# mcomunita/syncfusion

Hardware: AMD Instinct MI355X
Metric: U-Net denoise steps/sec (batch x 2 s@22.05 kHz) (higher is better)
Workload: dtype bf16; 1 GPU; BASELINE configs[1]: batch=8/GPU, 50-step DDIM (v-sampler) denoising of 2 s @ 22.05 kHz clips (L0=45056 = 44*1024, cropped to 44100), bf16, embedding_scale=1.0 (1 U-Net eval/step), dummy cond; this run timed 1568 consecutive sampler steps (the cost of a step does not depend on the schedule length); batch_per_gpu=8, L0=45056, hip_graph=True, weights_broadcast_bytes=0, gathered_clips=8

## Files before the change

include/syncfusion_amd.h:

```cpp
#ifndef SYNCFUSION_AMD_H
#define SYNCFUSION_AMD_H

#include <stdint.h>

#ifdef __cplusplus
extern "C" {
#endif

#define SF_MAX_DEPTH 12

enum {
  SF_OK = 0,
  SF_ERR_INVALID = 1,
  SF_ERR_MISSING_WEIGHT = 2,
  SF_ERR_SHAPE = 3,
  SF_ERR_HIP = 4,
  SF_ERR_WORKSPACE = 5,
  SF_ERR_UNSUPPORTED = 6
};

enum { SF_UP_NEAREST_CONV3 = 0, SF_UP_TRANSPOSE = 1 };
enum { SF_F32 = 0, SF_BF16 = 1, SF_F16 = 2, SF_F32X = 3 };

typedef struct {
// ... 24 lines not shown
  int32_t modulation_features;
  int32_t resnet_groups;
  int32_t dtype;
  int32_t upsample_mode;
  int32_t time_fourier_features, time_no_first_act, attention_out_bias;
} sf_unet_config;

typedef struct sf_unet sf_unet;

int sf_unet_create(const sf_unet_config *cfg, const sf_tensor *weights, int n_weights, void *stream, sf_unet **out);
void sf_unet_destroy(sf_unet *h);

int sf_unet_param_count(const sf_unet_config *cfg);
int sf_unet_param_name(const sf_unet_config *cfg, int index, char *name_out, int name_cap, int64_t *numel_out);

int64_t sf_unet_workspace_bytes(const sf_unet *h, int B, int L0, int two_pass);
int64_t sf_vsample_workspace_bytes(const sf_unet *h, int B, int L0, int two_pass, int num_steps);

int sf_unet_forward(sf_unet *h, const float *x, const float *sigma, const float *const *ctx, const float *emb,
                    int B, int L0, float embedding_scale, float *out, void *ws, int64_t ws_bytes, void *stream);

int sf_vsample(sf_unet *h, float *x_inout, const float *const *ctx, const float *emb, int B, int L0,
               int num_steps, float embedding_scale, int use_graph, void *ws, int64_t ws_bytes, void *stream);

int sf_unet_debug_enable(sf_unet *h, float *buf, int64_t cap_floats);
int sf_unet_debug_count(const sf_unet *h);
int sf_unet_debug_info(const sf_unet *h, int i, char *name_out, int name_cap, int64_t *offset, int64_t *rows, int32_t *cols);

int sf_unet_launch_count(const sf_unet *h);
int sf_unet_graph_captures(const sf_unet *h);
int sf_unet_set_branches(sf_unet *h, int n);
int sf_unet_profile_enable(sf_unet *h, int on);
int sf_unet_profile_count(const sf_unet *h);
int sf_unet_profile_get(const sf_unet *h, int i, char *name_out, int name_cap, float *ms, double *flops, double *bytes);
int sf_unet_profile_depth(const sf_unet *h, int i);

typedef struct {
  int32_t n_layers;
  int32_t in_channels;
  int32_t channels;
  int32_t multipliers[SF_MAX_DEPTH + 1];
  int32_t factors[SF_MAX_DEPTH];
  int32_t num_blocks[SF_MAX_DEPTH];
  int32_t resnet_groups;
  int32_t patch_size;
} sf_encoder1d_config;

typedef struct sf_encoder1d sf_encoder1d;

int sf_encoder1d_create(const sf_encoder1d_config *cfg, const sf_tensor *weights, int n_weights, void *stream, sf_encoder1d **out);
void sf_encoder1d_destroy(sf_encoder1d *h);
int64_t sf_encoder1d_workspace_bytes(const sf_encoder1d *h, int B, int L0);
int sf_encoder1d_forward(sf_encoder1d *h, const float *y, int B, int L0, float *const *xs_out,
                         void *ws, int64_t ws_bytes, void *stream);

typedef struct sf_onsetnet sf_onsetnet;

int sf_onsetnet_create(const sf_tensor *weights, int n_weights, int dtype, void *stream, sf_onsetnet **out);
void sf_onsetnet_destroy(sf_onsetnet *h);
int64_t sf_onsetnet_workspace_bytes(const sf_onsetnet *h, int N, int T, int H, int W);
int sf_onsetnet_forward(sf_onsetnet *h, const float *frames, int N, int T, int H, int W, float *logits,
                        void *ws, int64_t ws_bytes, void *stream);
int sf_onsetnet_debug_enable(sf_onsetnet *h, float *buf, int64_t cap_floats);
int sf_onsetnet_debug_count(const sf_onsetnet *h);
int sf_onsetnet_debug_info(const sf_onsetnet *h, int i, char *name_out, int name_cap, int64_t *offset, int64_t *rows, int32_t *cols);
int sf_onsetnet_debug_detail(sf_onsetnet *h, int enable, const int32_t *clips, int n_clips);
#define SF_ONSET_PATH_GEMM 0
#define SF_ONSET_PATH_GEMM_SPLIT 1
#define SF_ONSET_PATH_SP 2
#define SF_ONSET_PATH_TW 3
#define SF_ONSET_PATH_STEM 4
int sf_onsetnet_debug_path(const sf_onsetnet *h, int i);

int sf_onsets_to_track(const float *logits, int N, int T, const int32_t *start_frame ,
                       float frame_rate, float sample_rate, float threshold, float *track, int L, void *stream);

int sf_cut_prefix_crop(const float *gen, const float *y, int B, int C, int L, int cut_length, float *out, int32_t *first_onset,
                       void *stream);

typedef struct sf_resampler sf_resampler;
int sf_resampler_create(int orig_freq, int new_freq, int lowpass_filter_width, float rolloff, sf_resampler **out);
void sf_resampler_destroy(sf_resampler *h);
int sf_resampler_out_length(const sf_resampler *h, int L);
int sf_resampler_forward(sf_resampler *h, const float *x, int R, int L, float *out, void *stream);

typedef struct sf_augment_clip {
  int32_t top, left;
  int32_t order[4];
  float factor[4];
  int32_t mask;
  int32_t reserved;
} sf_augment_clip;
int64_t sf_frames_augment_workspace_bytes(int N, int T, int out_h, int out_w);
int sf_frames_augment(const uint8_t *frames, int N, int T, int H, int W, int resize_h, int resize_w, int out_h, int out_w,
                      const sf_augment_clip *table_host, const sf_augment_clip *table_dev, const float *mean3, const float *std3, float *out,
                      void *ws, int64_t ws_bytes, void *stream);
int sf_frames_preprocess(const uint8_t *frames, int N, int T, int H, int W, int out_h, int out_w, const float *mean3, const float *std3,
                         float *out, void *stream);
int sf_times_to_track(const double *times, const int32_t *clip_of, int n_times, double sample_rate, int B, int L, float *track, void *stream);

int sf_op_conv1d_cl(int dtype, const void *x, const float *w, const float *bias, const float *gamma, const float *beta,
                    int groups, float eps, const void *residual, int B, int L, int C, int N, int taps, int stride,
                    int pad, int upsample, void *out, void *ws, int64_t ws_bytes, void *stream);
int64_t sf_op_conv1d_bwd_workspace_bytes(int B, int L, int C, int N, int taps, int groups);
int sf_op_conv1d_bwd_cl(const float *x, const float *w, const float *gamma, const float *beta, int groups, float eps, const float *dy,
                        int B, int L, int C, int N, int taps, int pad, float *dx, float *dw, float *db, float *dgb, void *ws,
                        int64_t ws_bytes, void *stream);
int64_t sf_op_gn_silu_train_stats_floats(int B, int L, int C, int groups);
int sf_op_gn_silu_train(const float *x, const float *gamma, const float *beta, int groups, float eps, int B, int L, int C, float *act, float *stats,
                        void *stream);
int sf_op_conv1d_bwd_cl_act(const float *x, const float *act, const float *stats , const float *w, const float *gamma, const float *beta,
                            int groups, float eps, const float *dy, int B, int L, int C, int N, int taps, int pad, float *dx, float *dw, float *db,
                            float *dgb, void *ws, int64_t ws_bytes, void *stream);
int sf_op_conv1d_bwd_cl_x(int dtype, const float *x, const float *act, const float *stats, const float *w, const float *gamma, const float *beta,
                          int groups, float eps, const float *dy, int B, int L, int C, int N, int taps, int pad, float *dx, float *dw, float *db,
                          float *dgb, void *ws, int64_t ws_bytes, void *stream);
int64_t sf_op_conv1d_dgrad_pack_bytes(int C, int N, int taps);
int sf_op_conv1d_train_fwd(int dtype, const float *x, const float *w, const float *bias, const float *gamma, const float *beta, int groups, float eps,
                           const float *residual, int B, int L, int C, int N, int taps, int pad, float *out, void *dgrad_pack, int64_t dgrad_pack_bytes,
                           void *ws, int64_t ws_bytes, void *stream);
int sf_op_conv1d_bwd_cl_p(int dtype, const float *x, const float *act, const float *stats, const float *w, const void *dgrad_pack, const float *gamma,
                          const float *beta, int groups, float eps, const float *dy, const float *dx_add, int B, int L, int C, int N, int taps, int pad,
                          float *dx, float *dw, float *db, float *dgb, void *ws, int64_t ws_bytes, void *stream);
int sf_op_conv1d_train_images(int dtype, const float *w, int B, int L, int C, int N, int taps, int pad, int groups);
int sf_op_conv1d_variant(int dtype, int B, int L, int C, int N, int taps, int stride, int pad, int upsample, int groups, char *label, int label_bytes);
int sf_op_conv1d_bwd_variant(int dtype, int B, int L, int C, int N, int taps, int pad, char *label, int label_bytes);
int sf_train_pack_many(const void *desc_dev, int n_items, int total_tiles, void *stream);
int sf_op_conv1d_train_fwd_pk(int dtype, const float *x, const float *w, const float *fw, const void *fwx, const float *bias, const float *gamma,
                              const float *beta, int groups, float eps, const float *residual, int B, int L, int C, int N, int taps, int pad, float *out,
                              void *ws, int64_t ws_bytes, void *stream);
int sf_op_ln_modulate_bwd_add(const float *x, const float *scale_shift, const float *dy, const float *dx_add, float eps, int B, int L, int C, float *dx,
                              float *dss, void *ws, int64_t ws_bytes, void *stream);
int64_t sf_op_length_sums_workspace_bytes(int B, int L, int C);
int sf_op_length_sums(const float *x, const float *y , int B, int L, int C, float *out , void *ws, int64_t ws_bytes,
                      void *stream);
int64_t sf_op_ln_modulate_bwd_workspace_bytes(int B, int L, int C);
int sf_op_ln_modulate_bwd(const float *x, const float *scale_shift, const float *dy, float eps, int B, int L, int C, float *dx, float *dss,
                          void *ws, int64_t ws_bytes, void *stream);
int sf_op_attention_bwd(const float *q, const float *kv, const float *out, const float *dout, int B, int L, int heads, int head_dim, float *dq,
                        float *dkv, void *ws, int64_t ws_bytes, void *stream);
int sf_op_attention_fwd_lse(const float *q, const float *kv, int B, int L, int heads, int head_dim, float *out, float *lse, void *stream);
int sf_op_attention_fwd_lse_x(int dtype, const float *q, const float *kv, int B, int L, int heads, int head_dim, float *out, float *lse, void *stream);
int sf_op_attention_bwd_lse(const float *q, const float *kv, const float *out, const float *dout, const float *lse, int B, int L, int heads, int head_dim,
                            float *dq, float *dkv, void *ws, int64_t ws_bytes, void *stream);
int sf_op_attention_bwd_lse_x(int dtype, const float *q, const float *kv, const float *out, const float *dout, const float *lse, int B, int L, int heads,
                              int head_dim, float *dq, float *dkv, void *ws, int64_t ws_bytes, void *stream);
int sf_bench_conv1d(int dtype, int B, int L, int C, int N, int taps, int upsample, int path, int tile, int sk, int iters,
                    float *ms_out);
int64_t sf_op_resnet_mod_cb_workspace_bytes(int B, int L, int C);
int sf_op_resnet_mod_cb(int dtype, const void *x, const float *w1, const float *b1, const float *w2, const float *b2, const float *gn1_g,
                        const float *gn1_b, const float *gn2_g, const float *gn2_b, int groups, float eps_gn, const float *scale_shift,
                        float eps_ln, int B, int L, int C, int kb , void *h_out, void *m_out,
                        void *ws, int64_t ws_bytes, void *stream);
int64_t sf_op_inject_prenorm_proj_workspace_bytes(int B, int L, int C, int C2, int N);
int sf_op_inject_prenorm_proj(int dtype, const void *m, const void *ctx, const float *w_inj, const float *b_inj, const float *gamma,
                              const float *beta, float eps, const float *w_q, int B, int L, int C, int C2, int N, void *z_out, void *q_out,
                              int *fused_out, void *ws, int64_t ws_bytes, void *stream);
int sf_bench_conv_cb(int dtype, int B, int L, int C, int groups, int kb, int cold, int iters, float *ms );
int sf_op_gn_silu(int dtype, const void *x, const float *gamma, const float *beta, int groups, float eps, int B, int L, int C, void *out,
                  void *ws, int64_t ws_bytes, void *stream);
int sf_op_ln_modulate(int dtype, const void *x, const float *scale_shift , float eps,
                      int B, int L, int C, void *out, void *stream);
int sf_op_attention(int dtype, const void *q, const void *kv, int B, int L, int heads, int head_dim, void *out, void *stream);


typedef struct {
  int32_t N, T, Hi, Wi;
  int32_t cin, cin_ld;
  int32_t cout, cout_ld;
  int32_t kt, kh, kw;
  int32_t sh, sw;
  int32_t pt, ph, pw;
} sf_vconv_desc;
int64_t sf_op_vconv_workspace_bytes(const sf_vconv_desc *desc );
int sf_op_vconv_fwd(const sf_vconv_desc *desc, const float *x, const float *w, float *y, void *ws, int64_t ws_bytes, void *stream);
int sf_op_vconv_bwd(const sf_vconv_desc *desc, const float *x, const float *w, const float *dy, float *dx, float *dw, void *ws, int64_t ws_bytes,
                    void *stream);
int64_t sf_op_bn_train_workspace_bytes(int64_t rows, int C);
int sf_op_bn_train_fwd(const float *x, const float *res, int64_t rows, int C, int ld, const float *gamma, const float *beta, float eps, float momentum,
                       float *running_mean, float *running_var, int64_t *num_batches_tracked, int relu, float *y, float *save_mean, float *save_invstd,
                       void *ws, int64_t ws_bytes, void *stream);
int sf_op_bn_train_bwd(const float *x, const float *y, const float *dy, int64_t rows, int C, int ld, const float *gamma, const float *save_mean,
                       const float *save_invstd, float *dx, float *dres, float *dgamma, float *dbeta, void *ws, int64_t ws_bytes, void *stream);
int64_t sf_op_bn_sync_workspace_bytes(int64_t rows, int C);
int sf_op_bn_sync_stats(const float *x, int64_t rows, int C, int ld, float *local_stats, void *ws, int64_t ws_bytes, void *stream);
int sf_op_bn_sync_fwd_apply(const float *x, const float *res, int64_t rows, int C, int ld, const float *gathered_stats, const int64_t *row_counts, int world,
                            const float *gamma, const float *beta, float eps, float momentum, float *running_mean, float *running_var,
                            int64_t *num_batches_tracked, int relu, float *y, float *save_mean, float *save_invstd, void *ws, int64_t ws_bytes,
                            void *stream);
int sf_op_bn_sync_bwd_sums(const float *x, const float *y, const float *dy, int64_t rows, int C, int ld, const float *save_mean, const float *save_invstd,
                           float *local_sums, float *dgamma, float *dbeta, void *ws, int64_t ws_bytes, void *stream);
int sf_op_bn_sync_bwd_apply(const float *x, const float *y, const float *dy, int64_t rows, int C, int ld, const float *gathered_sums,
                            const int64_t *row_counts, int world, const float *gamma, const float *save_mean, const float *save_invstd, float *dx,
                            float *dres, void *ws, int64_t ws_bytes, void *stream);
int sf_op_video_to_cl(const float *x, int N, int C, int T, int H, int W, int ld, float *out, void *stream);
int sf_op_video_pool(const float *x, int64_t NT, int HW, int C, int ld, float *out, void *stream);
int sf_op_video_pool_bwd(const float *dout, int64_t NT, int HW, int C, int ld, float *dx, void *stream);

int64_t sf_op_onset_loss_workspace_bytes(int64_t n);
int sf_op_onset_bce_fwd(const float *z, const float *t, int64_t n, float *loss, float *stats, void *ws, int64_t ws_bytes, void *stream);
int sf_op_onset_bce_bwd(const float *z, const float *t, const float *stats, const float *g, int64_t n, float *dz, void *stream);
int sf_op_onset_metrics(const float *z, const float *t, int N, int T, float threshold, double *out, void *ws, int64_t ws_bytes, void *stream);

#define SF_OPTIM_CHUNK 16384
int64_t sf_optim_workspace_bytes(int total_chunks);
int sf_optim_adamw_step(const void *desc_dev, int n_tensors, int total_chunks, const void *hyper_dev, int n_groups, int clip, float *result_dev,
                        void *ws, int64_t ws_bytes, void *stream);

typedef struct sf_audio_features sf_audio_features;
enum { SF_PAD_CONSTANT = 0, SF_PAD_REFLECT = 1 };
int sf_audio_features_create(int n_fft, int hop, int n_mels, int pad_mode, const int32_t *first_bin , const int32_t *bin_count ,
                             const float *weights , int64_t n_weights, sf_audio_features **out);
void sf_audio_features_destroy(sf_audio_features *h);
int64_t sf_audio_features_workspace_bytes(const sf_audio_features *h, int B, int L);
int sf_logmel_forward(sf_audio_features *h, const float *wav, int B, int L, float amin, float top_db, float *mel_power, float *db, void *ws,
                      int64_t ws_bytes, void *stream);
int sf_onset_detect(sf_audio_features *h, const float *wav, int B, int L, float amin, float top_db, int lag, int pre_max, int post_max,
                    int pre_avg, int post_avg, int wait, float delta, int conf_interval, int capacity, float *envelope, int32_t *count,
                    int32_t *positions, float *confidence, float *strength, void *ws, int64_t ws_bytes, void *stream);

#ifdef __cplusplus
}
#endif
#endif
```

syncfusion_amd/_lib.py:

```python
from __future__ import annotations

import ctypes as C
import os
from typing import Dict, Iterable, List, Optional, Sequence, Tuple

import torch

SF_MAX_DEPTH = 12
SF_F32, SF_BF16, SF_F16, SF_F32X = 0, 1, 2, 3
UPSAMPLE_MODES = {"nearest": 0, "transpose": 1}
DTYPES = {"fp32": SF_F32, "float32": SF_F32, "f32": SF_F32, "bf16": SF_BF16, "bfloat16": SF_BF16, "fp16": SF_F16, "float16": SF_F16, "f16": SF_F16, "half": SF_F16,
          "fp32x": SF_F32X}

_HERE = os.path.dirname(os.path.abspath(__file__))
LIB_PATH = os.environ.get("SF_LIB_PATH") or os.path.join(_HERE, "lib", "libsyncfusion_amd.so")


class SfTensor(C.Structure):
    _fields_ = [("name", C.c_char_p), ("data", C.c_void_p), ("numel", C.c_int64)]


class UnetConfig(C.Structure):
    _fields_ = [
        ("n_layers", C.c_int32), ("in_channels", C.c_int32),
        ("channels", C.c_int32 * SF_MAX_DEPTH), ("factors", C.c_int32 * SF_MAX_DEPTH),
        ("items", C.c_int32 * SF_MAX_DEPTH), ("attentions", C.c_int32 * SF_MAX_DEPTH),
        ("cross_attentions", C.c_int32 * SF_MAX_DEPTH), ("context_channels", C.c_int32 * SF_MAX_DEPTH),
        ("attention_heads", C.c_int32), ("attention_features", C.c_int32),
        ("embedding_features", C.c_int32), ("embedding_max_length", C.c_int32),
        ("modulation_features", C.c_int32), ("resnet_groups", C.c_int32), ("dtype", C.c_int32),
        ("upsample_mode", C.c_int32),
        ("time_fourier_features", C.c_int32), ("time_no_first_act", C.c_int32), ("attention_out_bias", C.c_int32),
    ]


class EncoderConfig(C.Structure):
    _fields_ = [
        ("n_layers", C.c_int32), ("in_channels", C.c_int32), ("channels", C.c_int32),
        ("multipliers", C.c_int32 * (SF_MAX_DEPTH + 1)), ("factors", C.c_int32 * SF_MAX_DEPTH),
        ("num_blocks", C.c_int32 * SF_MAX_DEPTH), ("resnet_groups", C.c_int32), ("patch_size", C.c_int32),
    ]


class VConvDesc(C.Structure):
    _fields_ = [(n, C.c_int32) for n in ("N", "T", "Hi", "Wi", "cin", "cin_ld", "cout", "cout_ld", "kt", "kh", "kw", "sh", "sw", "pt", "ph", "pw")]


_P, _I, _L, _F = C.c_void_p, C.c_int, C.c_int64, C.c_float
SYMBOLS = {
    "sf_version": (C.c_char_p, []),
    "sf_last_error": (C.c_char_p, []),
    "sf_device_ok": (_I, []),
    "sf_clock_probe_start": (_I, [C.c_double, _P]),
    "sf_clock_probe_read": (_I, [C.POINTER(C.c_double)]),
    "sf_unet_create": (_I, [C.POINTER(UnetConfig), C.POINTER(SfTensor), _I, _P, C.POINTER(_P)]),
    "sf_unet_destroy": (None, [_P]),
    "sf_unet_param_count": (_I, [C.POINTER(UnetConfig)]),
    "sf_unet_param_name": (_I, [C.POINTER(UnetConfig), _I, C.c_char_p, _I, C.POINTER(_L)]),
    "sf_unet_workspace_bytes": (_L, [_P, _I, _I, _I]),
    "sf_vsample_workspace_bytes": (_L, [_P, _I, _I, _I, _I]),
    "sf_unet_forward": (_I, [_P, _P, _P, C.POINTER(_P), _P, _I, _I, _F, _P, _P, _L, _P]),
    "sf_vsample": (_I, [_P, _P, C.POINTER(_P), _P, _I, _I, _I, _F, _I, _P, _L, _P]),
    "sf_unet_debug_enable": (_I, [_P, _P, _L]),
    "sf_unet_debug_count": (_I, [_P]),
    "sf_unet_debug_info": (_I, [_P, _I, C.c_char_p, _I, C.POINTER(_L), C.POINTER(_L), C.POINTER(C.c_int32)]),
    "sf_unet_launch_count": (_I, [_P]),
    "sf_unet_graph_captures": (_I, [_P]),
    "sf_unet_set_branches": (_I, [_P, _I]),
    "sf_unet_profile_enable": (_I, [_P, _I]),
    "sf_unet_profile_count": (_I, [_P]),
    "sf_unet_profile_get": (_I, [_P, _I, C.c_char_p, _I, C.POINTER(C.c_float), C.POINTER(C.c_double), C.POINTER(C.c_double)]),
    "sf_unet_profile_depth": (_I, [_P, _I]),
    "sf_encoder1d_create": (_I, [C.POINTER(EncoderConfig), C.POINTER(SfTensor), _I, _P, C.POINTER(_P)]),
    "sf_encoder1d_destroy": (None, [_P]),
    "sf_encoder1d_workspace_bytes": (_L, [_P, _I, _I]),
    "sf_encoder1d_forward": (_I, [_P, _P, _I, _I, C.POINTER(_P), _P, _L, _P]),
    "sf_onsetnet_create": (_I, [C.POINTER(SfTensor), _I, _I, _P, C.POINTER(_P)]),
    "sf_onsetnet_destroy": (None, [_P]),
    "sf_onsetnet_workspace_bytes": (_L, [_P, _I, _I, _I, _I]),
    "sf_onsetnet_forward": (_I, [_P, _P, _I, _I, _I, _I, _P, _P, _L, _P]),
    "sf_onsetnet_debug_enable": (_I, [_P, _P, _L]),
    "sf_onsetnet_debug_count": (_I, [_P]),
    "sf_onsetnet_debug_detail": (_I, [_P, _I, C.POINTER(C.c_int32), _I]),
    "sf_onsetnet_debug_path": (_I, [_P, _I]),
    "sf_onsetnet_debug_info": (_I, [_P, _I, C.c_char_p, _I, C.POINTER(_L), C.POINTER(_L), C.POINTER(C.c_int32)]),
    "sf_onsets_to_track": (_I, [_P, _I, _I, _P, _F, _F, _F, _P, _I, _P]),
    "sf_frames_preprocess": (_I, [_P, _I, _I, _I, _I, _I, _I, _P, _P, _P, _P]),
    "sf_frames_augment_workspace_bytes": (_L, [_I, _I, _I, _I]),
    "sf_frames_augment": (_I, [_P, _I, _I, _I, _I, _I, _I, _I, _I, _P, _P, _P, _P, _P, _P, _L, _P]),
    "sf_times_to_track": (_I, [_P, _P, _I, C.c_double, _I, _I, _P, _P]),
    "sf_cut_prefix_crop": (_I, [_P, _P, _I, _I, _I, _I, _P, _P, _P]),
    "sf_resampler_create": (_I, [_I, _I, _I, _F, C.POINTER(_P)]),
    "sf_resampler_destroy": (None, [_P]),
    "sf_resampler_out_length": (_I, [_P, _I]),
    "sf_resampler_forward": (_I, [_P, _P, _I, _I, _P, _P]),
    "sf_op_conv1d_cl": (_I, [_I, _P, _P, _P, _P, _P, _I, _F, _P, _I, _I, _I, _I, _I, _I, _I, _I, _P, _P, _L, _P]),
    "sf_op_conv1d_bwd_workspace_bytes": (_L, [_I, _I, _I, _I, _I, _I]),
    "sf_op_conv1d_bwd_cl": (_I, [_P, _P, _P, _P, _I, _F, _P, _I, _I, _I, _I, _I, _I, _P, _P, _P, _P, _P, _L, _P]),
    "sf_op_conv1d_bwd_cl_act": (_I, [_P, _P, _P, _P, _P, _P, _I, _F, _P, _I, _I, _I, _I, _I, _I, _P, _P, _P, _P, _P, _L, _P]),
    "sf_op_conv1d_bwd_cl_x": (_I, [_I, _P, _P, _P, _P, _P, _P, _I, _F, _P, _I, _I, _I, _I, _I, _I, _P, _P, _P, _P, _P, _L, _P]),
    "sf_op_conv1d_dgrad_pack_bytes": (_L, [_I, _I, _I]),
    "sf_op_conv1d_train_fwd": (_I, [_I, _P, _P, _P, _P, _P, _I, _F, _P, _I, _I, _I, _I, _I, _I, _P, _P, _L, _P, _L, _P]),
    "sf_op_conv1d_bwd_cl_p": (_I, [_I, _P, _P, _P, _P, _P, _P, _P, _I, _F, _P, _P, _I, _I, _I, _I, _I, _I, _P, _P, _P, _P, _P, _L, _P]),
    "sf_op_conv1d_train_images": (_I, [_I, _P, _I, _I, _I, _I, _I, _I, _I]),
    "sf_op_conv1d_variant": (_I, [_I, _I, _I, _I, _I, _I, _I, _I, _I, _I, C.c_char_p, _I]),
    "sf_op_conv1d_bwd_variant": (_I, [_I, _I, _I, _I, _I, _I, _I, C.c_char_p, _I]),
    "sf_train_pack_many": (_I, [_P, _I, _I, _P]),
    "sf_op_conv1d_train_fwd_pk": (_I, [_I, _P, _P, _P, _P, _P, _P, _P, _I, _F, _P, _I, _I, _I, _I, _I, _I, _P, _P, _L, _P]),
    "sf_op_ln_modulate_bwd_add": (_I, [_P, _P, _P, _P, _F, _I, _I, _I, _P, _P, _P, _L, _P]),
    "sf_op_gn_silu_train_stats_floats": (_L, [_I, _I, _I, _I]),
    "sf_op_gn_silu_train": (_I, [_P, _P, _P, _I, _F, _I, _I, _I, _P, _P, _P]),
    "sf_op_ln_modulate_bwd_workspace_bytes": (_L, [_I, _I, _I]),
    "sf_op_ln_modulate_bwd": (_I, [_P, _P, _P, _F, _I, _I, _I, _P, _P, _P, _L, _P]),
    "sf_op_attention_bwd": (_I, [_P, _P, _P, _P, _I, _I, _I, _I, _P, _P, _P, _L, _P]),
    "sf_op_attention_fwd_lse": (_I, [_P, _P, _I, _I, _I, _I, _P, _P, _P]),
    "sf_op_attention_fwd_lse_x": (_I, [_I, _P, _P, _I, _I, _I, _I, _P, _P, _P]),
    "sf_op_attention_bwd_lse": (_I, [_P, _P, _P, _P, _P, _I, _I, _I, _I, _P, _P, _P, _L, _P]),
    "sf_op_attention_bwd_lse_x": (_I, [_I, _P, _P, _P, _P, _P, _I, _I, _I, _I, _P, _P, _P, _L, _P]),
    "sf_op_length_sums_workspace_bytes": (_L, [_I, _I, _I]),
    "sf_op_length_sums": (_I, [_P, _P, _I, _I, _I, _P, _P, _L, _P]),
    "sf_bench_conv1d": (_I, [_I, _I, _I, _I, _I, _I, _I, _I, _I, _I, _I, C.POINTER(C.c_float)]),
    "sf_op_gn_silu": (_I, [_I, _P, _P, _P, _I, _F, _I, _I, _I, _P, _P, _L, _P]),
    "sf_op_inject_prenorm_proj_workspace_bytes": (_L, [_I, _I, _I, _I, _I]),
    "sf_op_inject_prenorm_proj": (_I, [_I, _P, _P, _P, _P, _P, _P, _F, _P, _I, _I, _I, _I, _I, _P, _P, _P, _P, _L, _P]),
    "sf_op_resnet_mod_cb_workspace_bytes": (_L, [_I, _I, _I]),
    "sf_op_resnet_mod_cb": (_I, [_I, _P, _P, _P, _P, _P, _P, _P, _P, _P, _I, _F, _P, _F, _I, _I, _I, _I, _P, _P, _P, _L, _P]),
    "sf_bench_conv_cb": (_I, [_I, _I, _I, _I, _I, _I, _I, _I, C.POINTER(C.c_float)]),
    "sf_op_ln_modulate": (_I, [_I, _P, _P, _F, _I, _I, _I, _P, _P]),
    "sf_op_attention": (_I, [_I, _P, _P, _I, _I, _I, _I, _P, _P]),
    "sf_op_vconv_workspace_bytes": (_L, [C.POINTER(VConvDesc)]),
    "sf_op_vconv_fwd": (_I, [C.POINTER(VConvDesc), _P, _P, _P, _P, _L, _P]),
    "sf_op_vconv_bwd": (_I, [C.POINTER(VConvDesc), _P, _P, _P, _P, _P, _P, _L, _P]),
    "sf_op_bn_train_workspace_bytes": (_L, [_L, _I]),
    "sf_op_bn_train_fwd": (_I, [_P, _P, _L, _I, _I, _P, _P, _F, _F, _P, _P, _P, _I, _P, _P, _P, _P, _L, _P]),
    "sf_op_bn_train_bwd": (_I, [_P, _P, _P, _L, _I, _I, _P, _P, _P, _P, _P, _P, _P, _P, _L, _P]),
    "sf_op_bn_sync_workspace_bytes": (_L, [_L, _I]),
    "sf_op_bn_sync_stats": (_I, [_P, _L, _I, _I, _P, _P, _L, _P]),
    "sf_op_bn_sync_fwd_apply": (_I, [_P, _P, _L, _I, _I, _P, _P, _I, _P, _P, _F, _F, _P, _P, _P, _I, _P, _P, _P, _P, _L, _P]),
    "sf_op_bn_sync_bwd_sums": (_I, [_P, _P, _P, _L, _I, _I, _P, _P, _P, _P, _P, _P, _L, _P]),
    "sf_op_bn_sync_bwd_apply": (_I, [_P, _P, _P, _L, _I, _I, _P, _P, _I, _P, _P, _P, _P, _P, _P, _L, _P]),
    "sf_op_video_to_cl": (_I, [_P, _I, _I, _I, _I, _I, _I, _P, _P]),
    "sf_op_video_pool": (_I, [_P, _L, _I, _I, _I, _P, _P]),
    "sf_op_video_pool_bwd": (_I, [_P, _L, _I, _I, _I, _P, _P]),
    "sf_op_onset_loss_workspace_bytes": (_L, [_L]),
    "sf_op_onset_bce_fwd": (_I, [_P, _P, _L, _P, _P, _P, _L, _P]),
    "sf_op_onset_bce_bwd": (_I, [_P, _P, _P, _P, _L, _P, _P]),
    "sf_op_onset_metrics": (_I, [_P, _P, _I, _I, _F, _P, _P, _L, _P]),
    "sf_optim_workspace_bytes": (_L, [_I]),
    "sf_optim_adamw_step": (_I, [_P, _I, _I, _P, _I, _I, _P, _P, _L, _P]),
    "sf_audio_features_create": (_I, [_I, _I, _I, _I, _P, _P, _P, _L, C.POINTER(_P)]),
    "sf_audio_features_destroy": (None, [_P]),
    "sf_audio_features_workspace_bytes": (_L, [_P, _I, _I]),
    "sf_logmel_forward": (_I, [_P, _P, _I, _I, _F, _F, _P, _P, _P, _L, _P]),
    "sf_onset_detect": (_I, [_P, _P, _I, _I, _F, _F, _I, _I, _I, _I, _I, _I, _F, _I, _I, _P, _P, _P, _P, _P, _P, _L, _P]),
}

_lib: Optional[C.CDLL] = None


class SyncFusionAmdError(RuntimeError):
    pass


def load() -> C.CDLL:
    global _lib
    if _lib is not None:
        return _lib
    if not os.path.exists(LIB_PATH):
        raise SyncFusionAmdError(
            f"{LIB_PATH} is missing: build it with `python -c 'import __graft_entry__ as g; g.build()'` "
            "(or `make -C syncfusion_amd/csrc`).  There is no CPU fallback.")
    lib = C.CDLL(LIB_PATH)
    for name, (res, args) in SYMBOLS.items():
        fn = getattr(lib, name)
        fn.restype = res
        fn.argtypes = args
    _lib = lib
    return lib


def check(rc: int, what: str) -> None:
    if rc != 0:
        msg = load().sf_last_error()
        raise SyncFusionAmdError(f"{what} failed (code {rc}): {msg.decode() if msg else '?'}")


def require_gpu_tensor(t: torch.Tensor, where: str) -> None:
    if not t.is_cuda:
        raise SyncFusionAmdError(f"{where}: expected a tensor on an MI355X (cuda/hip) device, got {t.device}; "
                                 "this build has no CPU execution path")


def stream_ptr(device: torch.device) -> int:
    return int(torch.cuda.current_stream(device).cuda_stream)


def f32c(t: torch.Tensor) -> torch.Tensor:
    return t.detach().to(torch.float32).contiguous()


class TensorTable:

    def __init__(self, named: Iterable[Tuple[str, torch.Tensor]], device: torch.device):
        self.keep: List[torch.Tensor] = []
        self.names: List[bytes] = []
        items = list(named)
        self.array = (SfTensor * max(1, len(items)))()
        self.n = len(items)
        for i, (name, t) in enumerate(items):
            tt = f32c(t).to(device)
            self.keep.append(tt)
            self.names.append(name.encode())
            self.array[i].name = self.names[-1]
            self.array[i].data = tt.data_ptr()
            self.array[i].numel = tt.numel()


def ptr_array(tensors: Sequence[torch.Tensor]):
    arr = (C.c_void_p * len(tensors))()
    for i, t in enumerate(tensors):
        arr[i] = t.data_ptr()
    return arr
```

syncfusion_amd/csrc/capi_misc.cpp:

```cpp
#include <algorithm>
#include <cstring>
#include <cstdlib>
#include <cmath>
#include <exception>

#include "engine_common.h"

using namespace sf;

#define SF_API_BEGIN try {
#define SF_API_END                  \
  }                                 \
  catch (const EngineError &e) {    \
    return e.code;                  \
  }                                 \
  catch (const std::exception &e) { \
    set_error("%s", e.what());      \
    return SF_ERR_INVALID;          \
  }

extern "C" {

const char *sf_version(void) { return "syncfusion_amd 0.1.0 (gfx950)"; }
const char *sf_last_error(void) { return get_error(); }
// ... 372 lines not shown
  if (!ms_out || iters < 1) fail(SF_ERR_INVALID, "bad argument");
  const bool x3 = dtype == SF_F32X;
  if (x3) dtype = F32;
  const size_t es = dsize(dtype);
  const int K = taps * C, Lout = L * upsample, M = B * Lout;
  void *x = nullptr, *w = nullptr, *out = nullptr, *res = nullptr;
  float *bias = nullptr;
  SF_HIP(hipMalloc(&x, (size_t)B * L * C * es));
  const size_t wbytes = (size_t)N * K * es;
  int ncopy = 1;
  if (const char *e = tune_env("SF_BENCH_COLD")) {
    if (atoi(e) > 0) ncopy = (int)std::min<size_t>(1024, ((size_t)768 << 20) / wbytes + 1);
  }
  SF_HIP(hipMalloc(&w, wbytes * ncopy));
  SF_HIP(hipMalloc(&out, (size_t)M * N * es));
  SF_HIP(hipMalloc(&res, (size_t)M * N * es));
  SF_HIP(hipMalloc(&bias, N * sizeof(float)));
  SF_HIP(hipMemset(x, 0x3c, (size_t)B * L * C * es));
  SF_HIP(hipMemset(w, 0xbc, wbytes * ncopy));
  SF_HIP(hipMemset(res, 0x3d, (size_t)M * N * es));
  SF_HIP(hipMemset(bias, 0, N * sizeof(float)));
  ConvGemmArgs a;
  a.src = x;
  a.src_ld = C;
  a.w = w;
  a.bias = bias;
  a.N = N;
  a.K = K;
  a.cin = C;
  a.taps = taps;
  a.pad = taps / 2;
  while ((1 << a.up_shift) < upsample) ++a.up_shift;
  a.Lsrc = L;
  a.Lout = Lout;
  a.M = M;
  a.out = out;
  a.out_ld = N;
  a.n_store = N;
  a.res = res;
  a.res_ld = N;
  g_conv_gemm_force.path = path;
  g_conv_gemm_force.tile = tile;
  g_conv_gemm_force.sk = sk;
  hipEvent_t e0, e1;
  SF_HIP(hipEventCreate(&e0));
  SF_HIP(hipEventCreate(&e1));
  hipError_t err = hipSuccess;
  unsigned *sink = nullptr;
  void *wfr = nullptr;
  if (dtype != F32 && (K % 64) == 0 && K <= 2048 && (N % 32) == 0 && (C % 16) == 0 && !tune_env("SF_BENCH_NO_WFR")) {
    SF_HIP(hipMalloc(&wfr, wbytes * ncopy));
    SF_HIP(hipMemcpy(wfr, w, wbytes * ncopy, hipMemcpyDeviceToDevice));
    a.wfr = wfr;
  }
  void *wx = nullptr;
  if (x3) {
    if (K % 32) fail(SF_ERR_UNSUPPORTED, "fp32x needs K %% 32 == 0");
    SF_HIP(hipMalloc(&wx, wbytes * ncopy));
    for (int c = 0; c < ncopy; ++c)
      SF_HIP(launch_pack_wx(reinterpret_cast<const float *>(static_cast<char *>(w) + (size_t)c * wbytes), N, K, static_cast<char *>(wx) + (size_t)c * wbytes, nullptr));
    a.wx = wx;
  }
  for (int i = 0; i < 3 && err == hipSuccess; ++i) err = launch_conv_gemm(dtype, a, nullptr);
  if (err == hipSuccess) {
    SF_HIP(hipDeviceSynchronize());
    SF_HIP(hipEventRecord(e0, nullptr));
    int pre = 0;
    if (const char *e = tune_env("SF_BENCH_PREFETCH")) pre = atoi(e);
    if (pre > 0 && pre % 1000 == 0) fail(SF_ERR_INVALID, "SF_BENCH_PREFETCH=%d: the workgroup count (value mod 1000) must be >= 1", pre);
    if (pre > 0) SF_HIP(hipMalloc(reinterpret_cast<void **>(&sink), 64));
    for (int i = 0; i < iters && err == hipSuccess; ++i) {
      a.w = static_cast<char *>(w) + (size_t)(i % ncopy) * wbytes;
      if (wfr) a.wfr = static_cast<char *>(wfr) + (size_t)(i % ncopy) * wbytes;
      if (wx) a.wx = static_cast<char *>(wx) + (size_t)(i % ncopy) * wbytes;
      if (pre > 0) err = launch_touch(a.w, wbytes, pre % 1000, sink, nullptr);
      if (pre < 1000 && err == hipSuccess) err = launch_conv_gemm(dtype, a, nullptr);
    }
    SF_HIP(hipEventRecord(e1, nullptr));
    SF_HIP(hipEventSynchronize(e1));
    SF_HIP(hipEventElapsedTime(ms_out, e0, e1));
    *ms_out /= (float)iters;
  }
  g_conv_gemm_force = ConvGemmForce();
  (void)hipEventDestroy(e0);
  (void)hipEventDestroy(e1);
  for (void *p : {x, w, out, res, (void *)bias}) (void)hipFree(p);
  if (sink) (void)hipFree(sink);
  if (wfr) (void)hipFree(wfr);
  if (wx) (void)hipFree(wx);
  if (err != hipSuccess) fail(SF_ERR_UNSUPPORTED, "variant not applicable: %s", hipGetErrorString(err));
  return SF_OK;
  SF_API_END
}

int64_t sf_op_resnet_mod_cb_workspace_bytes(int B, int L, int C) {
  Workspace dry(nullptr, 0);
  const int64_t M = (int64_t)B * L;
  dry.alloc(2 * (int64_t)C * C * 3 * 4);
  dry.alloc(M * C * 4);
  dry.alloc(M * C * 4);
  dry.alloc((int64_t)(C / 128) * M * C * 4);
  dry.alloc((int64_t)B * 32 * 64 * 2 * 4);
  return dry.used();
}

int sf_op_resnet_mod_cb(int dtype, const void *x, const float *w1, const float *b1, const float *w2, const float *b2, const float *gn1_g,
                        const float *gn1_b, const float *gn2_g, const float *gn2_b, int groups, float eps_gn, const float *scale_shift, float eps_ln,
                        int B, int L, int C, int kb, void *h_out, void *m_out, void *ws, int64_t ws_bytes, void *stream) {
  SF_API_BEGIN
  if (kb != 1 && kb != 2) fail(SF_ERR_INVALID, "kb must be 1 or 2");
  if (!x || !w1 || !b1 || !w2 || !b2 || !gn1_g || !gn1_b || !gn2_g || !gn2_b || !m_out || !ws) fail(SF_ERR_INVALID, "null argument");
  if (!conv_cb_shape_ok(dtype, B, L, C, C, groups) || groups > 64) fail(SF_ERR_UNSUPPORTED, "shape outside the channel-block convolution's coverage");
  hipStream_t s = static_cast<hipStream_t>(stream);
  Workspace wk(ws, ws_bytes);
  const int64_t M = (int64_t)B * L;
  const int S = C / 128 / kb;
  if (kb == 2 && ((C / 128) % 2 || C / groups < 32)) fail(SF_ERR_UNSUPPORTED, "two channel blocks per workgroup need C a multiple of 256 and >= 32 channels per group");
  if (kb == 2 && dtype == SF_F32X) fail(SF_ERR_UNSUPPORTED, "the split-operand form takes one channel block per workgroup");
  const int64_t es = (int64_t)dsize(dtype);
  const int adt = dtype == SF_F32X ? (int)F32 : dtype;
  char *wp = static_cast<char *>(wk.alloc(2 * (int64_t)C * C * 3 * es));
  void *wp1 = wp, *wp2 = wp + (int64_t)C * C * 3 * es;
  void *act = wk.alloc(M * C * es);
  void *h = h_out ? h_out : wk.alloc(M * C * es);
  float *slab = static_cast<float *>(wk.alloc((int64_t)S * M * C * 4));
  float *stats = static_cast<float *>(wk.alloc((int64_t)B * 32 * 64 * 2 * 4));
  SF_HIP(launch_pack_conv_cb(dtype, w1, C, C, wp1, s));
  SF_HIP(launch_pack_conv_cb(dtype, w2, C, C, wp2, s));
  SF_HIP(launch_gn_silu(adt, x, C, B, L, C, groups, gn1_g, gn1_b, eps_gn, act, C, s));
  ConvCbArgs a;
  a.src = act;
  a.src_ld = C;
  a.wp = wp1;
  a.slab = slab;
  a.B = B;
  a.L = L;
  a.C = a.N = C;
  a.kb = kb;
  SF_HIP(launch_conv_cb(dtype, a, s));
  const CbGnPlan gp = cb_gn_plan(L);
  SF_HIP(launch_cb_reduce_gn(adt, slab, S, B, L, C, b1, h, C, groups, stats, gp, s));
  a.src = h;
  a.wp = wp2;
  a.pro = 1;
  a.G = groups;
  a.nch = gp.nch;
  a.chunk_rows = gp.chunk_rows;
  a.stats = stats;
  a.gamma = gn2_g;
  a.beta = gn2_b;
  a.eps = eps_gn;
  SF_HIP(launch_conv_cb(dtype, a, s));
  SF_HIP(launch_cb_reduce_ln(adt, slab, S, B, L, C, b2, x, C, scale_shift, 2 * C, eps_ln, m_out, C, s));
  return SF_OK;
  SF_API_END
}

int64_t sf_op_inject_prenorm_proj_workspace_bytes(int B, int L, int C, int C2, int N) {
  if (B < 1 || L < 1 || C < 32 || C2 < 0 || N < 8) return -1;
  const int64_t M = (int64_t)B * L, K1 = C + (C2 + 31) / 32 * 32;
  return (int64_t)C * K1 * 2 + (int64_t)N * C * 2 + M * C * 2 + M * (C / 32) * 8 + (int64_t)(2 * N + C) * 4 + 4096;
}

int sf_op_inject_prenorm_proj(int dtype, const void *m, const void *ctx, const float *w_inj, const float *b_inj, const float *gamma,
                              const float *beta, float eps, const float *w_q, int B, int L, int C, int C2, int N, void *z_out, void *q_out,
                              int *fused_out, void *ws, int64_t ws_bytes, void *stream) {
  SF_API_BEGIN
  if (!m || !w_inj || !b_inj || !gamma || !beta || !w_q || !z_out || !q_out || !ws) fail(SF_ERR_INVALID, "null argument");
  if (dtype != BF16 && dtype != F16) fail(SF_ERR_UNSUPPORTED, "16-bit dtypes only");
  if (C % 32 || C2 % 32 || N % 32 || (C2 > 0 && !ctx)) fail(SF_ERR_UNSUPPORTED, "C, C2 and N must be multiples of 32");
  const int64_t need = sf_op_inject_prenorm_proj_workspace_bytes(B, L, C, C2, N);
  if (need < 0 || ws_bytes < need) fail(SF_ERR_WORKSPACE, "workspace too small: need %lld bytes", (long long)need);
  hipStream_t s = static_cast<hipStream_t>(stream);
  Workspace wk(ws, ws_bytes);
  const int64_t M = (int64_t)B * L;
  const int K1 = C + C2;
  void *w1 = wk.alloc((int64_t)C * K1 * 2), *w2 = wk.alloc((int64_t)N * C * 2), *tmp = wk.alloc(M * C * 2);
  float *rowpart = static_cast<float *>(wk.alloc(M * (C / 32) * 8));
  float *bias2 = static_cast<float *>(wk.alloc((int64_t)N * 4)), *colsum = static_cast<float *>(wk.alloc((int64_t)N * 4));
  SF_HIP(launch_pack_rows(dtype, w_inj, C, K1, K1, nullptr, w1, K1, s));
  SF_HIP(launch_pack_rows(dtype, w_q, N, C, C, gamma, w2, C, s));
  SF_HIP(launch_fold_bias(w_q, N, C, beta, nullptr, bias2, s));
  SF_HIP(launch_row_sums(dtype, w2, N, C, colsum, s));
  ConvGemmArgs a;
  a.src = m;
  a.src_ld = C;
  a.src2 = ctx;
  a.src2_ld = C2;
  a.w = w1;
  a.bias = b_inj;
  a.M = (int)M;
  a.N = a.n_store = C;
  a.K = K1;
  a.cin = C;
  a.cin2 = C2;
  a.taps = 1;
  a.Lout = a.Lsrc = L;
  a.out = z_out;
  a.out_ld = C;
  a.res = m;
  a.res_ld = C;
  ConvGemmArgs q;
  q.src = z_out;
  q.src_ld = C;
  q.w = w2;
  q.bias = bias2;
  q.M = (int)M;
  q.N = q.n_store = N;
  q.K = q.cin = C;
  q.taps = 1;
  q.Lout = q.Lsrc = L;
  q.out = q_out;
  q.out_ld = N;
  ConvGemmArgs ar = a, ql = q;
  ar.rowpart_out = rowpart;
  ar.rowpart_nt = C / 32;
  ql.ln_part = rowpart;
  ql.ln_nt = C / 32;
  ql.ln_eps = eps;
  ql.ln_colsum = colsum;
  ar.mt_ln = ql.mt_ln = 1;
  const bool fused = conv_gemm_emits_rowpart(dtype, ar) && conv_gemm_ln_ok(dtype, ql);
  if (fused_out) *fused_out = fused ? 1 : 0;
  if (fused) {
    SF_HIP(launch_conv_gemm(dtype, ar, s));
    SF_HIP(launch_conv_gemm_ln(dtype, ql, s));
  } else {
    if (!conv_gemm_supported(dtype, a) || !conv_gemm_supported(dtype, q)) fail(SF_ERR_UNSUPPORTED, "shape outside the GEMM kernels' coverage");
    SF_HIP(launch_conv_gemm(dtype, a, s));
    SF_HIP(launch_ln_modulate(dtype, z_out, C, nullptr, 0, eps, B, L, C, tmp, C, s));
    q.src = tmp;
    SF_HIP(launch_conv_gemm(dtype, q, s));
  }
  return SF_OK;
  SF_API_END
}

int sf_bench_conv_cb(int dtype, int B, int L, int C, int groups, int kb, int cold, int iters, float *ms) {
  SF_API_BEGIN
  if (!ms || iters < 1 || (kb != 1 && kb != 2)) fail(SF_ERR_INVALID, "bad argument");
  if (!conv_cb_shape_ok(dtype, B, L, C, C, groups)) fail(SF_ERR_UNSUPPORTED, "shape outside the channel-block convolution's coverage");
  const int64_t M = (int64_t)B * L;
  const int S = C / 128 / kb;
  const size_t wbytes = (size_t)C * C * 3 * 2;
  int ncopy = 1;
  if (cold) ncopy = (int)std::min<size_t>(256, (768u << 20) / wbytes + 1);
  void *w = nullptr, *x = nullptr, *h = nullptr;
  float *slab = nullptr, *stats = nullptr, *vec = nullptr;
  SF_HIP(hipMalloc(&w, wbytes * ncopy));
  SF_HIP(hipMalloc(&x, M * C * 2));
  SF_HIP(hipMalloc(&h, M * C * 2));
  SF_HIP(hipMalloc(reinterpret_cast<void **>(&slab), (size_t)S * M * C * 4));
  SF_HIP(hipMalloc(reinterpret_cast<void **>(&stats), (size_t)B * 32 * 64 * 2 * 4));
  SF_HIP(hipMalloc(reinterpret_cast<void **>(&vec), (size_t)(4 * C + (size_t)B * 2 * C) * 4));
  SF_HIP(hipMemset(w, 0x11, wbytes * ncopy));
  SF_HIP(hipMemset(x, 0x3c, M * C * 2));
  SF_HIP(hipMemset(vec, 0, (size_t)(4 * C + (size_t)B * 2 * C) * 4));
  const CbGnPlan gp = cb_gn_plan(L);
  ConvCbArgs a;
  a.src = x;
  a.src_ld = C;
  a.slab = slab;
  a.B = B;
  a.L = L;
  a.C = a.N = C;
  a.kb = kb;
  a.G = groups;
  a.nch = gp.nch;
  a.chunk_rows = gp.chunk_rows;
  a.stats = stats;
  a.gamma = vec;
  a.beta = vec + C;
  hipEvent_t e0, e1;
  SF_HIP(hipEventCreate(&e0));
  SF_HIP(hipEventCreate(&e1));
  hipError_t err = hipSuccess;
  for (int which = 0; which < 4 && err == hipSuccess; ++which) {
    auto one = [&](int i) -> hipError_t {
      a.wp = static_cast<char *>(w) + (size_t)(i % ncopy) * wbytes;
      switch (which) {
        case 0: a.pro = 0; return launch_conv_cb(dtype, a, nullptr);
        case 1: return launch_cb_reduce_gn(dtype, slab, S, B, L, C, vec + 2 * C, h, C, groups, stats, gp, nullptr);
        case 2: a.pro = 1; return launch_conv_cb(dtype, a, nullptr);
        default: return launch_cb_reduce_ln(dtype, slab, S, B, L, C, vec + 2 * C, x, C, vec + 4 * C, 2 * C, 1e-6f, h, C, nullptr);
      }
    };
    for (int i = 0; i < 3 && err == hipSuccess; ++i) err = one(i);
    if (err != hipSuccess) break;
    SF_HIP(hipDeviceSynchronize());
    SF_HIP(hipEventRecord(e0, nullptr));
    for (int i = 0; i < iters && err == hipSuccess; ++i) err = one(i);
    SF_HIP(hipEventRecord(e1, nullptr));
    SF_HIP(hipEventSynchronize(e1));
    SF_HIP(hipEventElapsedTime(&ms[which], e0, e1));
    ms[which] /= (float)iters;
  }
  (void)hipEventDestroy(e0);
  (void)hipEventDestroy(e1);
  for (void *p : {w, x, h, (void *)slab, (void *)stats, (void *)vec}) (void)hipFree(p);
  if (err != hipSuccess) fail(SF_ERR_HIP, "launch failed: %s", hipGetErrorString(err));
  return SF_OK;
  SF_API_END
}

int sf_op_ln_modulate(int dtype, const void *x, const float *scale_shift, float eps, int B, int L, int C, void *out, void *stream) {
  SF_API_BEGIN
// ... 19 lines not shown
```

syncfusion_amd/csrc/conv_cb.hip:

```cpp
#include <cstdlib>

#include "common.h"
#include "kernels.h"

namespace sf {
namespace {

constexpr int KC = 128;
constexpr int KC_LOG2 = 7;
constexpr int NSLOT = 4;
constexpr unsigned OOB = 0x80000000u;

template <typename T> __device__ __forceinline__ Vec16<T> buf_ld16(__amdgpu_buffer_rsrc_t r, unsigned byte_off) {
  Vec16<T> v;
  u32x4 raw = __builtin_amdgcn_raw_buffer_load_b128(r, byte_off, 0, 0);
  v.v = __builtin_bit_cast(decltype(v.v), raw);
  return v;
}

__device__ __forceinline__ float part_count(bool tiles, int clip, int kc, int mtile, int L, int chunk_rows, int log2cpg) {
  const int c0 = clip * L;
  const int rows = tiles ? min((mtile + 1) * 32, c0 + L) - max(mtile * 32, c0) : min(chunk_rows, L - kc * chunk_rows);
  return (float)(rows << (tiles ? 5 : log2cpg));
}

__device__ __forceinline__ float2 merge_parts(const float2 (&cs)[4], const float (&cn)[4], int sub, int lim, float rn, float eps) {
  float s1 = 0.f;
#pragma unroll
  for (int k = 0; k < 4; ++k)
    if (sub + 8 * k < lim) s1 = fmaf(cn[k], cs[k].x, s1);
  const float mean = sum8_dpp(s1) * rn;
  float s2 = 0.f;
#pragma unroll
  for (int k = 0; k < 4; ++k)
    if (sub + 8 * k < lim) {
      const float d = cs[k].x - mean;
      s2 += fmaf(cn[k] * d, d, cs[k].y);
    }
  return make_float2(mean, rsqrtf(sum8_dpp(s2) * rn + eps));
}

template <typename T, int MT, bool PRO, int KB>
__global__ __launch_bounds__(256) void conv_cb_kernel(const ConvCbArgs a, const int mtiles, const unsigned bytes_src) {
  using frag = typename Frag16<T>::type;
  constexpr int KCW = KC * KB, PITCHW = KCW + 8, TPR = KCW / 8, RPP = 256 / TPR;
  constexpr int BM = 32 * MT, PR = BM + 2, NV = (PR + RPP - 1) / RPP;
  __shared__ __attribute__((aligned(16))) T panel[PR * PITCHW];
  __shared__ float2 gstat[NSLOT][8];
  const int tid = threadIdx.x, lane = tid & 63;
  const int wave = __builtin_amdgcn_readfirstlane(tid >> 6);
  const int nws = (int)gridDim.x;
  if ((int)blockIdx.y >= mtiles) {
    prefetch_slice(a.pf, ((int)blockIdx.y - mtiles) * nws + (int)blockIdx.x, 256);
    return;
  }
  const int mt = (int)blockIdx.y, ws = (int)blockIdx.x;
  const int nt = ws >> a.log2S, cb = ws & ((1 << a.log2S) - 1);
  const int r0 = mt * BM, M = a.B * a.L;
  auto divL = [&](int x) { return (int)__umulhi((unsigned)x, a.magicL); };

  const __amdgpu_buffer_rsrc_t rS = __builtin_amdgcn_make_buffer_rsrc(const_cast<void *>(a.src), 0, bytes_src, 0x00020000);
  const int cv = tid % TPR, pr = tid / TPR;
  Vec16<T> pv[NV];
  const unsigned col_b = (unsigned)((cb * KCW + cv * 8) * sizeof(T)), row_b = (unsigned)(a.src_ld * sizeof(T));
#pragma unroll
  for (int i = 0; i < NV; ++i) {
    const int j = pr + RPP * i, r = r0 - 1 + j;
    const bool ok = j < PR && r >= 0 && r < M;
    pv[i] = buf_ld16<T>(rS, ok ? (unsigned)r * row_b + col_b : OOB);
  }
  const int gshift = KC_LOG2 + (KB == 2 ? 1 : 0) - a.log2cpg;
  const int clip0 = divL(max(r0 - 1, 0));
  const int nclip = PRO ? (divL(min(r0 + BM, M - 1)) - clip0 + 1) : 0;
  const int npair = nclip << gshift;
  f32x4 ga[2], be[2];
  constexpr int NRD = 1;
  float2 cs[NRD][4];
  float cn[NRD][4];
  int lim[NRD] = {0};
  const int sub = tid & 7;
  if constexpr (PRO) {
    const int G = a.C >> a.log2cpg;
#pragma unroll
    for (int q = 0; q < 2; ++q) {
      ga[q] = *reinterpret_cast<const f32x4 *>(a.gamma + cb * KCW + cv * 8 + 4 * q);
      be[q] = *reinterpret_cast<const f32x4 *>(a.beta + cb * KCW + cv * 8 + 4 * q);
    }
    const bool tiles = a.pro == 2;
    const int ltpg = a.log2cpg - 5, ct = a.C >> 5;
#pragma unroll
    for (int rd = 0; rd < NRD; ++rd) {
      const int p = min((tid >> 3) + 32 * rd, npair - 1);
      const int slot = p >> gshift, gi = p & ((1 << gshift) - 1);
      const int clip = clip0 + slot;
      const int mt_lo = (clip * a.L) >> 5, nmt = ((clip * a.L + a.L - 1) >> 5) - mt_lo + 1;
      lim[rd] = tiles ? (nmt << max(ltpg, 0)) : a.nch;
#pragma unroll
      for (int k = 0; k < 4; ++k) {
        const int kc = min(sub + 8 * k, lim[rd] - 1);
        const int mtile = mt_lo + (kc >> max(ltpg, 0));
        const int tile = (((cb << gshift) + gi) << max(ltpg, 0)) + (kc & ((1 << max(ltpg, 0)) - 1));
        const unsigned off2 = (unsigned)(((mtile * ct + tile) * 2 + (clip - divL(mtile << 5))) * 2);
        const unsigned off1 = (unsigned)((((clip * a.nch + kc) * G) + (cb << gshift) + gi) * 2);
        cs[rd][k] = *reinterpret_cast<const float2 *>(a.stats + (tiles ? off2 : off1));
        cn[rd][k] = part_count(tiles, clip, kc, mtile, a.L, a.chunk_rows, a.log2cpg);
      }
    }
  }
  __builtin_amdgcn_sched_barrier(0);
  frag wf[24 * KB];
#pragma unroll
  for (int blk = 0; blk < KB; ++blk) {
    const frag *wp = reinterpret_cast<const frag *>(a.wp) + ((size_t)((cb * KB + blk) * (a.N >> 5) + (nt * 4 + wave)) * 24) * 64;
#pragma unroll
    for (int s = 0; s < 24; ++s) wf[blk * 24 + s] = wp[s * 64 + lane];
  }
  __builtin_amdgcn_sched_barrier(0);
  if constexpr (PRO) {
#pragma unroll
    for (int rd = 0; rd < NRD; ++rd)
#pragma unroll
      for (int k = 0; k < 4; ++k) asm volatile("" : "+v"(cs[rd][k].x), "+v"(cs[rd][k].y));
  }
  if constexpr (PRO) {
    const float rn = 1.0f / ((float)a.L * (float)(1 << a.log2cpg));
#pragma unroll
    for (int rd = 0; rd < NRD; ++rd) {
      const float2 st = merge_parts(cs[rd], cn[rd], sub, lim[rd], rn, a.eps);
      const int p = (tid >> 3) + 32 * rd;
      if (sub == 0 && p < npair) gstat[p >> gshift][p & ((1 << gshift) - 1)] = st;
    }
    __syncthreads();
  }
#pragma unroll
  for (int i = 0; i < NV; ++i) {
    const int j = pr + RPP * i, r = r0 - 1 + j;
    if (j < PR) {
      Vec16<T> o = pv[i];
      if (PRO && r >= 0 && r < M) {
        const float2 st = gstat[divL(r) - clip0][(cv * 8) >> a.log2cpg];
#pragma unroll
        for (int e = 0; e < 8; ++e) {
          const float sc = st.y * ga[e >> 2][e & 3];
          const float sh = fmaf(-st.x, sc, be[e >> 2][e & 3]);
          o.set(e, silu_t<true>(fmaf(pv[i].get(e), sc, sh)));
        }
      }
      st16<T>(panel + j * PITCHW + cv * 8, o);
    }
  }
  __syncthreads();
  const int fr = lane & 31, fh = lane >> 5;
  bool ok0[MT], ok2[MT];
#pragma unroll
  for (int t = 0; t < MT; ++t) {
    const int m = r0 + t * 32 + fr, l = m - divL(m) * a.L;
    ok0[t] = l > 0;
    ok2[t] = l < a.L - 1;
  }
  f32x16 acc[MT];
#pragma unroll
  for (int t = 0; t < MT; ++t)
#pragma unroll
    for (int r = 0; r < 16; ++r) acc[t][r] = 0.f;
  const frag zf = __builtin_bit_cast(frag, u32x4{0u, 0u, 0u, 0u});
#pragma unroll
  for (int blk = 0; blk < KB; ++blk)
#pragma unroll
    for (int tap = 0; tap < 3; ++tap)
#pragma unroll
      for (int ks = 0; ks < 8; ++ks)
#pragma unroll
        for (int t = 0; t < MT; ++t) {
          frag af = *reinterpret_cast<const frag *>(panel + (t * 32 + fr + tap) * PITCHW + blk * KC + ks * 16 + fh * 8);
          if (tap == 0) af = ok0[t] ? af : zf;
          if (tap == 2) af = ok2[t] ? af : zf;
          acc[t] = mfma32x16(wf[blk * 24 + tap * 8 + ks], af, acc[t]);
        }
  float *sl = a.slab + (size_t)cb * M * a.N + nt * 128 + wave * 32 + 4 * fh;
#pragma unroll
  for (int t = 0; t < MT; ++t) {
    const int m = r0 + t * 32 + fr;
    if (m < M) {
#pragma unroll
      for (int g = 0; g < 4; ++g) {
        f32x4 v = {acc[t][4 * g], acc[t][4 * g + 1], acc[t][4 * g + 2], acc[t][4 * g + 3]};
        *reinterpret_cast<f32x4 *>(sl + (unsigned)(m * a.N + 8 * g)) = v;
      }
    }
  }
}

template <int MT, bool PRO>
__global__ __launch_bounds__(256) void conv_cb_x3_kernel(const ConvCbArgs a, const int mtiles, const unsigned bytes_src) {
  using frag = f16x8;
  constexpr int PITCHW = KC + 8, TPR = KC / 4, RPP = 256 / TPR;
  constexpr int BM = 32 * MT, PR = BM + 2, NV = (PR + RPP - 1) / RPP;
  __shared__ __attribute__((aligned(16))) f16 panelH[PR * PITCHW], panelL[PR * PITCHW];
  __shared__ float2 gstat[NSLOT][8];
  const int tid = threadIdx.x, lane = tid & 63;
  const int wave = __builtin_amdgcn_readfirstlane(tid >> 6);
  const int nws = (int)gridDim.x;
  if ((int)blockIdx.y >= mtiles) {
    prefetch_slice(a.pf, ((int)blockIdx.y - mtiles) * nws + (int)blockIdx.x, 256);
    return;
  }
  const int mt = (int)blockIdx.y, ws = (int)blockIdx.x;
  const int nt = ws >> a.log2S, cb = ws & ((1 << a.log2S) - 1);
  const int r0 = mt * BM, M = a.B * a.L;
  auto divL = [&](int x) { return (int)__umulhi((unsigned)x, a.magicL); };

  const __amdgpu_buffer_rsrc_t rS = __builtin_amdgcn_make_buffer_rsrc(const_cast<void *>(a.src), 0, bytes_src, 0x00020000);
  const int cv = tid % TPR, pr = tid / TPR;
  f32x4 pv[NV];
  const unsigned col_b = (unsigned)((cb * KC + cv * 4) * 4), row_b = (unsigned)(a.src_ld * 4);
#pragma unroll
  for (int i = 0; i < NV; ++i) {
    const int j = pr + RPP * i, r = r0 - 1 + j;
    const bool ok = j < PR && r >= 0 && r < M;
    pv[i] = __builtin_bit_cast(f32x4, __builtin_amdgcn_raw_buffer_load_b128(rS, ok ? (unsigned)r * row_b + col_b : OOB, 0, 0));
  }
  const int gshift = KC_LOG2 - a.log2cpg;
  const int clip0 = divL(max(r0 - 1, 0));
  const int nclip = PRO ? (divL(min(r0 + BM, M - 1)) - clip0 + 1) : 0;
  const int npair = nclip << gshift;
  f32x4 ga = {1.f, 1.f, 1.f, 1.f}, be = {0.f, 0.f, 0.f, 0.f};
  float2 cs[4];
  float cn[4];
  int lim = 0;
  const int sub = tid & 7;
  if constexpr (PRO) {
    const int G = a.C >> a.log2cpg;
    ga = *reinterpret_cast<const f32x4 *>(a.gamma + cb * KC + cv * 4);
    be = *reinterpret_cast<const f32x4 *>(a.beta + cb * KC + cv * 4);
    const bool tiles = a.pro == 2;
    const int ltpg = a.log2cpg - 5, ct = a.C >> 5;
    const int p = min(tid >> 3, npair - 1);
    const int slot = p >> gshift, gi = p & ((1 << gshift) - 1);
    const int clip = clip0 + slot;
    const int mt_lo = (clip * a.L) >> 5, nmt = ((clip * a.L + a.L - 1) >> 5) - mt_lo + 1;
    lim = tiles ? (nmt << max(ltpg, 0)) : a.nch;
#pragma unroll
    for (int k = 0; k < 4; ++k) {
      const int kc = min(sub + 8 * k, lim - 1);
      const int mtile = mt_lo + (kc >> max(ltpg, 0));
      const int tile = (((cb << gshift) + gi) << max(ltpg, 0)) + (kc & ((1 << max(ltpg, 0)) - 1));
      const unsigned off2 = (unsigned)(((mtile * ct + tile) * 2 + (clip - divL(mtile << 5))) * 2);
      const unsigned off1 = (unsigned)((((clip * a.nch + kc) * G) + (cb << gshift) + gi) * 2);
      cs[k] = *reinterpret_cast<const float2 *>(a.stats + (tiles ? off2 : off1));
      cn[k] = part_count(tiles, clip, kc, mtile, a.L, a.chunk_rows, a.log2cpg);
    }
  }
  __builtin_amdgcn_sched_barrier(0);
  frag wh[24], wl[24];
  {
    const frag *wp = reinterpret_cast<const frag *>(a.wp) + ((size_t)(cb * (a.N >> 5) + (nt * 4 + wave)) * 48) * 64;
#pragma unroll
    for (int s = 0; s < 24; ++s) {
      wh[s] = wp[(2 * s) * 64 + lane];
      wl[s] = wp[(2 * s + 1) * 64 + lane];
    }
  }
  __builtin_amdgcn_sched_barrier(0);
  if constexpr (PRO) {
#pragma unroll
    for (int k = 0; k < 4; ++k) asm volatile("" : "+v"(cs[k].x), "+v"(cs[k].y));
  }
  if constexpr (PRO) {
    const float rn = 1.0f / ((float)a.L * (float)(1 << a.log2cpg));
    const float2 st = merge_parts(cs, cn, sub, lim, rn, a.eps);
    const int p = tid >> 3;
    if (sub == 0 && p < npair) gstat[p >> gshift][p & ((1 << gshift) - 1)] = st;
    __syncthreads();
  }
  typedef f16 f16x4_c __attribute__((ext_vector_type(4)));
#pragma unroll
  for (int i = 0; i < NV; ++i) {
    const int j = pr + RPP * i, r = r0 - 1 + j;
    if (j < PR) {
      f32x4 o = pv[i];
      if (PRO && r >= 0 && r < M) {
        const float2 st = gstat[divL(r) - clip0][(cv * 4) >> a.log2cpg];
#pragma unroll
        for (int e = 0; e < 4; ++e) {
          const float sc = st.y * ga[e];
          const float sh = fmaf(-st.x, sc, be[e]);
          o[e] = silu_t<false>(fmaf(pv[i][e], sc, sh));
        }
      }
      f16x4_c h, l;
#pragma unroll
      for (int e = 0; e < 4; ++e) {
        f16 x, y;
        x3_split1<X3_F16>(o[e], x, y);
        h[e] = x;
        l[e] = y;
      }
      *reinterpret_cast<f16x4_c *>(panelH + j * PITCHW + cv * 4) = h;
      *reinterpret_cast<f16x4_c *>(panelL + j * PITCHW + cv * 4) = l;
    }
  }
  __syncthreads();
  const int fr = lane & 31, fh = lane >> 5;
  bool ok0[MT], ok2[MT];
#pragma unroll
  for (int t = 0; t < MT; ++t) {
    const int m = r0 + t * 32 + fr, l = m - divL(m) * a.L;
    ok0[t] = l > 0;
    ok2[t] = l < a.L - 1;
  }
  f32x16 acc[MT], accL[MT];
#pragma unroll
  for (int t = 0; t < MT; ++t)
#pragma unroll
    for (int r = 0; r < 16; ++r) acc[t][r] = accL[t][r] = 0.f;
  const frag zf = __builtin_bit_cast(frag, u32x4{0u, 0u, 0u, 0u});
#pragma unroll
  for (int tap = 0; tap < 3; ++tap)
#pragma unroll
    for (int ks = 0; ks < 8; ++ks)
#pragma unroll
      for (int t = 0; t < MT; ++t) {
        const int o = (t * 32 + fr + tap) * PITCHW + ks * 16 + fh * 8;
        frag ah = *reinterpret_cast<const frag *>(panelH + o), al = *reinterpret_cast<const frag *>(panelL + o);
        if (tap == 0) {
          ah = ok0[t] ? ah : zf;
          al = ok0[t] ? al : zf;
        }
        if (tap == 2) {
          ah = ok2[t] ? ah : zf;
          al = ok2[t] ? al : zf;
        }
        x3_mfma<X3_F16>(wh[tap * 8 + ks], wl[tap * 8 + ks], ah, al, acc[t], accL[t]);
      }
  float *sl = a.slab + (size_t)cb * M * a.N + nt * 128 + wave * 32 + 4 * fh;
#pragma unroll
  for (int t = 0; t < MT; ++t) {
    const int m = r0 + t * 32 + fr;
    if (m < M) {
#pragma unroll
      for (int g = 0; g < 4; ++g) {
        f32x4 v;
// ... 65 lines not shown
  const f32x4 bi = *reinterpret_cast<const f32x4 *>(bias + c);
  float xs[P][4];
  float s1 = 0.f;
#pragma unroll
  for (int p = 0; p < P; ++p) {
    const int lr = p * 8 + rr;
    f32x4 x = v[p][0];
#pragma unroll
    for (int s = 1; s < S; ++s) x += v[p][s];
    x += bi;
    T o[4];
#pragma unroll
    for (int e = 0; e < 4; ++e) {
      o[e] = from_f<T>(x[e]);
      xs[p][e] = lr < rows ? to_f(o[e]) : 0.f;
      s1 += xs[p][e];
    }
    if (lr < rows) __builtin_memcpy(__builtin_assume_aligned(out + ((size_t)b * L + l0 + lr) * out_ld + c, 4 * sizeof(T)), o, 4 * sizeof(T));
  }
  const int cpg = N / G, span = cpg / 4;
  const int gpb = 128 / cpg;
  auto group_total = [&](float t, int k) {
    for (int off = 1; off < span; off <<= 1) t += __shfl_xor(t, off, 64);
    t += __shfl_xor(t, 32, 64);
    if (lane < 32 && (cq % span) == 0) red[wave][cq / span][k] = t;
    __syncthreads();
    float a = 0.f;
    if (tid < gpb) {
#pragma unroll
      for (int w = 0; w < 4; ++w) a += red[w][tid][k];
    }
    return a;
  };
  const float a1 = group_total(s1, 0);
  if (tid < gpb) gmean[tid] = a1 / ((float)rows * (float)cpg);
  __syncthreads();
  const float mu = gmean[cq / span];
  float s2 = 0.f;
#pragma unroll
  for (int p = 0; p < P; ++p) {
    const bool live = p * 8 + rr < rows;
#pragma unroll
    for (int e = 0; e < 4; ++e) {
      const float d = live ? xs[p][e] - mu : 0.f;
      s2 = fmaf(d, d, s2);
    }
  }
  const float a2 = group_total(s2, 1);
  if (tid < gpb) {
    float *o = stats + (((size_t)b * nch + ch) * G + cblk * gpb + tid) * 2;
    o[0] = gmean[tid];
    o[1] = a2;
  }
}

template <typename T, int S, int TPR>
__global__ __launch_bounds__(256) void cb_reduce_ln_kernel(const float *__restrict__ slab, const int M, const int C, const int L,
                                                           const float *__restrict__ bias, const T *__restrict__ res, const int res_ld,
                                                           const float *__restrict__ ss, const int ss_ld, const float eps, T *__restrict__ out,
                                                           const int out_ld, const int nreal, const Prefetch pf) {
  constexpr int RPB = 256 / TPR, WPR = TPR >= 64 ? TPR / 64 : 1;
  __shared__ float red[2][4];
  if ((int)blockIdx.x >= nreal) {
    prefetch_slice(pf, (int)blockIdx.x - nreal, 256);
    return;
  }
  const int tid = threadIdx.x, wave = tid >> 6;
  const int row = (int)blockIdx.x * RPB + tid / TPR, sub = tid % TPR;
  const bool active = row < M;
  const size_t m = active ? row : 0;
  const int c = sub * 4, b = (int)(m / L);
  f32x4 v[S];
#pragma unroll
  for (int s = 0; s < S; ++s) v[s] = *reinterpret_cast<const f32x4 *>(slab + ((size_t)s * M + m) * C + c);
  T rv[4];
  __builtin_memcpy(rv, __builtin_assume_aligned(res + m * res_ld + c, 4 * sizeof(T)), 4 * sizeof(T));
  const f32x4 bi = *reinterpret_cast<const f32x4 *>(bias + c);
  f32x4 sc = {0.f, 0.f, 0.f, 0.f}, sh = {0.f, 0.f, 0.f, 0.f};
  if (ss) {
    sc = *reinterpret_cast<const f32x4 *>(ss + (size_t)b * ss_ld + c);
    sh = *reinterpret_cast<const f32x4 *>(ss + (size_t)b * ss_ld + C + c);
  }
  f32x4 y = v[0];
#pragma unroll
  for (int s = 1; s < S; ++s) y += v[s];
  y += bi;
#pragma unroll
  for (int e = 0; e < 4; ++e) y[e] += to_f(rv[e]);
  auto row_sum = [&](float x, int slot) {
    constexpr int W = TPR < 64 ? TPR : 64;
#pragma unroll
    for (int o = W >> 1; o > 0; o >>= 1) x += __shfl_xor(x, o, 64);
    if constexpr (WPR > 1) {
      if ((tid & 63) == 0) red[slot][wave] = x;
      __syncthreads();
      const int w0 = (wave / WPR) * WPR;
      x = 0.f;
#pragma unroll
      for (int w = 0; w < WPR; ++w) x += red[slot][w0 + w];
    }
    return x;
  };
  const float mean = row_sum((y[0] + y[1]) + (y[2] + y[3]), 0) / (float)C;
  float q = 0.f;
#pragma unroll
  for (int e = 0; e < 4; ++e) {
    const float d = y[e] - mean;
    q = fmaf(d, d, q);
  }
  const float rstd = rsqrtf(row_sum(q, 1) / (float)C + eps);
  if (!active) return;
  T o[4];
#pragma unroll
  for (int e = 0; e < 4; ++e) {
    float z = (y[e] - mean) * rstd;
    if (ss) z = fmaf(z, 1.0f + sc[e], sh[e]);
    o[e] = from_f<T>(z);
  }
  __builtin_memcpy(__builtin_assume_aligned(out + (size_t)row * out_ld + c, 4 * sizeof(T)), o, 4 * sizeof(T));
}

int cb_min_wgs() {
  static const int v = [] {
    const char *e = tune_env("SF_CB_MIN_WGS");
    return e && atoi(e) > 0 ? atoi(e) : 160;
  }();
  return v;
}

}

size_t conv_cb_weight_elems(int N, int C) { return (size_t)N * C * 3; }

bool conv_cb_shape_ok(int dt, int B, int L, int C, int N, int G) {
  if (dt == F32) return false;
  if (C < KC || (C % KC) || (N % 128) || C / KC > 8 || ((C / KC) & (C / KC - 1))) return false;
  if (L < 44 || (int64_t)B * L * (int64_t)(C > N ? C : N) * 4 >= 0x7FFFFFF0ll) return false;
  if ((uint64_t)B * L * (uint64_t)L >= (1ull << 32)) return false;
  if (G > 0) {
    if (C % G) return false;
    const int cpg = C / G;
    if (cpg < 16 || cpg > KC || (cpg & (cpg - 1))) return false;
  }
  return true;
}

bool conv_cb_tile_stats_ok(int L, int C, int G) {
  if (G < 1 || C % G) return false;
  const int cpg = C / G;
  if (cpg < 32 || (cpg & (cpg - 1)) || L < 32) return false;
  return ((L + 30) / 32 + 1) * (cpg / 32) <= 32;
}

int conv_cb_mt(int M, int N, int C) {
  static const int forced = [] {
    const char *e = tune_env("SF_CB_MT");
    return e ? atoi(e) : 0;
  }();
  if (forced >= 1 && forced <= 4) return forced;
  const int nws = (N / 128) * (C / KC);
  return ((M + 63) / 64) * nws >= cb_min_wgs() ? 2 : 1;
}

hipError_t launch_pack_conv_cb(int dt, const float *w, int N, int C, void *out, hipStream_t s) {
  if (dt == F32 || (C % KC) || (N % 32)) return hipErrorInvalidValue;
  const size_t total = (size_t)N * C * 3;
  const int blocks = (int)std::min<size_t>((total + 255) / 256, 4096);
  if (dt == F32X) hipLaunchKernelGGL(pack_conv_cb_x3_kernel, dim3(blocks), dim3(256), 0, s, w, N, C, static_cast<f16 *>(out));
  else if (dt == BF16) hipLaunchKernelGGL((pack_conv_cb_kernel<bf16>), dim3(blocks), dim3(256), 0, s, w, N, C, static_cast<bf16 *>(out));
  else hipLaunchKernelGGL((pack_conv_cb_kernel<f16>), dim3(blocks), dim3(256), 0, s, w, N, C, static_cast<f16 *>(out));
  return hipGetLastError();
}

hipError_t launch_conv_cb(int dt, const ConvCbArgs &a0, hipStream_t s) {
  if (!conv_cb_shape_ok(dt, a0.B, a0.L, a0.C, a0.N, a0.pro ? a0.G : 0)) return hipErrorInvalidValue;
  if (a0.pro == 1 && a0.nch > 32) return hipErrorInvalidValue;
  if (a0.pro == 2 && !conv_cb_tile_stats_ok(a0.L, a0.C, a0.G)) return hipErrorInvalidValue;
  ConvCbArgs a = a0;
  if (dt == F32X && a.kb == 2) return hipErrorInvalidValue;
  const int kb = a.kb == 2 ? 2 : 1;
  const int M = a.B * a.L, S = a.C / KC / kb;
  if (kb == 2 && ((a.C / KC) % 2 || (a.pro && a.C / a.G < 32))) return hipErrorInvalidValue;
  a.log2S = 0;
  while ((1 << a.log2S) < S) ++a.log2S;
  const int cpg = a.pro ? a.C / a.G : KC;
  a.log2cpg = 0;
  while ((1 << a.log2cpg) < cpg) ++a.log2cpg;
  if ((1 << a.log2S) != S || (1 << a.log2cpg) != cpg) return hipErrorInvalidValue;
  a.magicL = (unsigned)((0x100000000ull + (unsigned)a.L - 1) / (unsigned)a.L);
  int mt = kb == 2 ? std::min(2, conv_cb_mt(M, a.N, a.C / 2)) : conv_cb_mt(M, a.N, a.C);
  if (dt == F32X) mt = std::min(mt, 2);
  const int mtiles = (M + 32 * mt - 1) / (32 * mt), nws = (a.N / 128) * S;
  const int pf_rows = (a.pf.ptr && a.pf.bytes >= 16 && a.pf.wgs > 0) ? (a.pf.wgs + nws - 1) / nws : 0;
  a.pf.wgs = pf_rows * nws;
  const dim3 grid(nws, mtiles + pf_rows);
  const unsigned bytes_src = (unsigned)((size_t)M * a.src_ld * dsize(dt));
  if (dt == F32X) {
    if (a.pro) {
      if (mt == 1) hipLaunchKernelGGL((conv_cb_x3_kernel<1, true>), grid, dim3(256), 0, s, a, mtiles, bytes_src);
      else hipLaunchKernelGGL((conv_cb_x3_kernel<2, true>), grid, dim3(256), 0, s, a, mtiles, bytes_src);
    } else {
      if (mt == 1) hipLaunchKernelGGL((conv_cb_x3_kernel<1, false>), grid, dim3(256), 0, s, a, mtiles, bytes_src);
      else hipLaunchKernelGGL((conv_cb_x3_kernel<2, false>), grid, dim3(256), 0, s, a, mtiles, bytes_src);
    }
    return hipGetLastError();
  }
#define SF_CB2(T, MT, KB_)                                                                                                \
  do {                                                                                                                    \
    if (a.pro) hipLaunchKernelGGL((conv_cb_kernel<T, MT, true, KB_>), grid, dim3(256), 0, s, a, mtiles, bytes_src);       \
    else hipLaunchKernelGGL((conv_cb_kernel<T, MT, false, KB_>), grid, dim3(256), 0, s, a, mtiles, bytes_src);            \
  } while (0)
#define SF_CB(T, MT)                 \
  do {                               \
    if (kb == 2) SF_CB2(T, MT, 2);   \
    else SF_CB2(T, MT, 1);           \
  } while (0)
#define SF_CB_T(T)            \
  switch (mt) {               \
    case 1: SF_CB(T, 1); break; \
    case 2: SF_CB(T, 2); break; \
    case 3: if (kb == 2) { SF_CB2(T, 2, 2); } else { SF_CB2(T, 3, 1); } break; \
    default: if (kb == 2) { SF_CB2(T, 2, 2); } else { SF_CB2(T, 4, 1); } break; \
  }
  if (dt == BF16) { SF_CB_T(bf16) } else { SF_CB_T(f16) }
#undef SF_CB_T
#undef SF_CB
#undef SF_CB2
  return hipGetLastError();
}

CbGnPlan cb_gn_plan(int L) {
  CbGnPlan p;
  int P = 1;
  while (P < 4 && (L + 8 * P - 1) / (8 * P) > 32) P *= 2;
  p.chunk_rows = 8 * P;
  p.nch = (L + p.chunk_rows - 1) / p.chunk_rows;
  return p;
}

hipError_t launch_cb_reduce_gn(int dt, const float *slab, int S, int B, int L, int N, const float *bias, void *out, int out_ld, int G, float *stats,
                               const CbGnPlan &gp, hipStream_t s, Prefetch pf) {
  if ((N % 128) || N % G || (N / G) < 16 || (N / G) > 128 || (128 % (N / G)) || gp.nch > 32 || (out_ld % 4)) return hipErrorInvalidValue;
  const int P = gp.chunk_rows / 8, M = B * L;
  const int nreal = B * gp.nch * (N / 128);
  const dim3 grid(nreal + (pf.ptr && pf.bytes >= 16 ? pf.wgs : 0));
#define SF_RG(T, S_, P_)                                                                                                                          \
  hipLaunchKernelGGL((cb_reduce_gn_kernel<T, S_, P_>), grid, dim3(256), 0, s, slab, M, N, L, bias, static_cast<T *>(out), out_ld, G, stats, gp.nch, \
                     nreal, pf)
#define SF_RG_P(T, S_)            \
  switch (P) {                    \
    case 1: SF_RG(T, S_, 1); break; \
    case 2: SF_RG(T, S_, 2); break; \
    case 4: SF_RG(T, S_, 4); break; \
    default: return hipErrorInvalidValue; \
  }
#define SF_RG_S(T)                \
  switch (S) {                    \
    case 1: SF_RG_P(T, 1) break;  \
    case 2: SF_RG_P(T, 2) break;  \
    case 4: SF_RG_P(T, 4) break;  \
    case 8: SF_RG_P(T, 8) break;  \
    default: return hipErrorInvalidValue; \
  }
  if (dt == BF16) { SF_RG_S(bf16) } else if (dt == F16) { SF_RG_S(f16) } else { SF_RG_S(float) }
#undef SF_RG_S
#undef SF_RG_P
#undef SF_RG
  return hipGetLastError();
}

hipError_t launch_cb_reduce_ln(int dt, const float *slab, int S, int B, int L, int C, const float *bias, const void *res, int res_ld, const float *ss,
                               int ss_ld, float eps, void *out, int out_ld, hipStream_t s, Prefetch pf) {
  const int tpr = C / 4;
  if ((C % 128) || (tpr != 32 && tpr != 64 && tpr != 128 && tpr != 256) || (res_ld % 4) || (out_ld % 4)) return hipErrorInvalidValue;
  if (ss && ((ss_ld % 4) || (reinterpret_cast<uintptr_t>(ss) % 16))) return hipErrorInvalidValue;
  const int M = B * L, rpb = 256 / tpr;
  const int nreal = (M + rpb - 1) / rpb;
  const dim3 grid(nreal + (pf.ptr && pf.bytes >= 16 ? pf.wgs : 0));
#define SF_RL(T, S_, TPR_)                                                                                                                     \
  hipLaunchKernelGGL((cb_reduce_ln_kernel<T, S_, TPR_>), grid, dim3(256), 0, s, slab, M, C, L, bias, static_cast<const T *>(res), res_ld, ss, ss_ld, \
                     eps, static_cast<T *>(out), out_ld, nreal, pf)
#define SF_RL_T(T, S_)               \
  switch (tpr) {                     \
    case 32: SF_RL(T, S_, 32); break;  \
    case 64: SF_RL(T, S_, 64); break;  \
    case 128: SF_RL(T, S_, 128); break; \
    default: SF_RL(T, S_, 256); break; \
  }
#define SF_RL_S(T)                 \
  switch (S) {                     \
    case 1: SF_RL_T(T, 1) break;   \
    case 2: SF_RL_T(T, 2) break;   \
    case 4: SF_RL_T(T, 4) break;   \
    case 8: SF_RL_T(T, 8) break;   \
    default: return hipErrorInvalidValue; \
  }
  if (dt == BF16) { SF_RL_S(bf16) } else if (dt == F16) { SF_RL_S(f16) } else { SF_RL_S(float) }
#undef SF_RL_S
#undef SF_RL_T
#undef SF_RL
  return hipGetLastError();
}

}
```

syncfusion_amd/csrc/conv_gemm.hip:

```cpp
#include <cstring>
#include <set>
#include <string>

#include "common.h"
#include "kernels.h"

namespace sf {

namespace {

constexpr int BK = 32;

template <typename T> struct Lds {
  static constexpr int LD = BK + 16 / (int)sizeof(T);
};

struct RowState {
  int valid_m;
  int b_rel;
  int p0;
  int base;
  int t, h, w;
};

// ... 274 lines not shown
        rv[r] = has_res ? to_f(res[(size_t)m * a.res_ld + nc]) : 0.f;
        const int b = has_b ? m / a.Lout : 0;
        sv[r] = has_bs ? a.bscale[(size_t)b * a.bscale_ld + nc] : 1.f;
        av[r] = has_ba ? a.badd[(size_t)b * a.badd_ld + nc] : 0.f;
      }
#pragma unroll
      for (int r = 0; r < 16; ++r) {
        const int m = m0 + wr * WTM + i * 32 + (r & 3) + 8 * (r >> 2) + 4 * fh;
        float v = (acc[i][j][r] + bias) * sv[r] + rv[r] + av[r];
        v = real ? apply_act(v, a.act) : 0.f;
        if (m < a.M && n < a.n_store) {
          if (a.out_f32) static_cast<float *>(a.out)[(size_t)m * a.out_ld + n] = v;
          else out[(size_t)m * a.out_ld + n] = from_f<T>(v);
        }
      }
    }
  }
}

template <typename T, int BM, int BN, int WM_, int WN_, bool SC>
hipError_t launch_cfg(const ConvGemmArgs &a, hipStream_t s) {
  constexpr int LD = Lds<T>::LD;
  size_t lds = (size_t)(BM + BN) * LD * sizeof(T);
  if (a.pro == 1) {
    int nb = min(a.M / a.Lout + (a.M % a.Lout ? 1 : 0), BM / a.Lout + 2);
    lds += (size_t)nb * (a.cin + a.G) * sizeof(float2);
  }
  dim3 grid((a.M + BM - 1) / BM, (a.n_store + BN - 1) / BN);
  auto kern = conv_gemm_kernel<T, BM, BN, WM_, WN_, SC>;
  static bool big_lds_enabled = false;
  if (!big_lds_enabled) {
    hipError_t e = hipFuncSetAttribute(reinterpret_cast<const void *>(kern), hipFuncAttributeMaxDynamicSharedMemorySize, 128 * 1024);
    if (e != hipSuccess) return e;
    big_lds_enabled = true;
  }
  hipLaunchKernelGGL(kern, grid, dim3(256), lds, s, a);
  return hipGetLastError();
}

int pick_variant(const ConvGemmArgs &a);
int pick_variant(const ConvGemmArgs &a) {
  if (g_conv_gemm_force.path == 1 && g_conv_gemm_force.tile >= 1 && g_conv_gemm_force.tile <= 4) return g_conv_gemm_force.tile;
  const bool scalar_a = (a.cin % BK) != 0 || (a.cin2 % BK) != 0;
  if (scalar_a) return (a.cin2 != 0 || a.pro != 0) ? -1 : 0;
  const long M = a.M, N = a.n_store;
  auto blocks = [&](int bm, int bn) { return ((M + bm - 1) / bm) * ((N + bn - 1) / bn); };
  if (N <= 32) return 1;
  if (N <= 64) return blocks(128, 64) >= 512 ? 2 : 3;
  if (blocks(128, 128) >= 512) return 4;
  if (blocks(128, 64) >= 384) return 2;
  return 3;
}

template <typename T> hipError_t dispatch(const ConvGemmArgs &a, hipStream_t s) {
  switch (pick_variant(a)) {
    case 0: return launch_cfg<T, 64, 64, 2, 2, true>(a, s);
    case 1: return launch_cfg<T, 128, 32, 4, 1, false>(a, s);
    case 2: return launch_cfg<T, 128, 64, 2, 2, false>(a, s);
    case 3: return launch_cfg<T, 64, 64, 2, 2, false>(a, s);
    case 4: return launch_cfg<T, 128, 128, 2, 2, false>(a, s);
    default: return hipErrorInvalidValue;
  }
}

}

bool conv_gemm_supported(int dt, const ConvGemmArgs &a) {
  (void)dt;
  if (a.M <= 0 || a.N <= 0 || a.K <= 0) return false;
  if (a.pro == 1) {
    if (a.geom != 0 || a.cin % BK || a.cin % a.G) return false;
    int nb = min(a.M / a.Lout + 1, 128 / a.Lout + 2);
    if ((size_t)nb * (a.cin + a.G) * 8 > 96 * 1024) return false;
  }
  return true;
}

hipError_t launch_conv_gemm_sk(int dt, const ConvGemmArgs &a, hipStream_t s);
int conv_gemm_sk_variant(const ConvGemmArgs &a);
bool conv_gemm_fast_ok(int dt, const ConvGemmArgs &a);
bool conv_gemm_wp_ok(int dt, const ConvGemmArgs &a);
bool conv_gemm_prefers_wp(const ConvGemmArgs &a);

static bool use_sk(const ConvGemmArgs &a) {
  const int v = pick_variant(a);
  if (v <= 0 || (a.K % 32)) return false;
  static const int bm[5] = {64, 128, 128, 64, 128}, bn[5] = {64, 32, 64, 64, 128};
  const long blocks = (long)((a.M + bm[v] - 1) / bm[v]) * ((a.n_store + bn[v] - 1) / bn[v]);
  return blocks < 256 && a.K >= 256;
}

const char *label_for_dtype(int dt, const char *bf16_label) {
  if (dt != F16) return bf16_label;
  static std::set<std::string> pool;
  std::string s(bf16_label);
  const size_t at = s.find("bf16");
  if (at != std::string::npos) s.replace(at, 4, "f16");
  return pool.insert(s).first->c_str();
}

static const char *variant_name_bf16(int dt, const ConvGemmArgs &a);
static const char *label_x3(const ConvGemmArgs &a, const char *f32_label) {
  if (!a.wx) return f32_label;
  std::string s(f32_label);
  if (s.rfind("conv_gemm_wp<f32", 0) != 0 && s.rfind("conv_gemm_fast<f32", 0) != 0) return f32_label;
  static std::set<std::string> pool;
  s.replace(s.find("f32"), 3, "x3");
  return pool.insert(s).first->c_str();
}
const char *conv_gemm_variant_name(int dt, const ConvGemmArgs &a) {
  return dt == F32 ? label_x3(a, variant_name_bf16(dt, a)) : label_for_dtype(dt, variant_name_bf16(dt, a));
}
bool conv_gemm_reads_split_only(int dt, const ConvGemmArgs &a_in) {
  ConvGemmArgs a = a_in;
  a.w = a.wx = reinterpret_cast<const void *>(16);
  return std::strstr(conv_gemm_variant_name(dt, a), "<x3") != nullptr;
}

static long short_act_tiles() {
  static const long v = [] {
    const char *e = tune_env("SF_SHORT_TILES");
    const long t = e ? atol(e) : 0;
    return t > 0 ? t : 500L;
  }();
  return v;
}

bool conv_gemm_prefers_mt(const ConvGemmArgs &a) {
  static const int mode = [] {
    const char *e = tune_env("SF_MT");
    return e ? atoi(e) : 1;
  }();
  if (mode == 0) return false;
  if (mode == 2) return true;
  static const int min_tiles = [] {
    const char *e = tune_env("SF_MT_TILES");
    const int v = e ? atoi(e) : 0;
    return v > 0 ? v : 40;
  }();
  if (a.n_store <= 64 && a.geom != 1) return false;
  const long tiles = (long)((a.M + 127) / 128) * ((a.n_store + 127) / 128);
  return tiles >= 2 * min_tiles && a.K >= (a.geom == 1 ? 128 : 256);
}

static const char *variant_name_bf16(int dt, const ConvGemmArgs &a) {
  if (g_conv_gemm_force.path == 6 || (g_conv_gemm_force.path == 0 && conv_gemm_mt_wanted(dt, a))) return dt == F32 ? (a.wx ? "conv_gemm_mt<x3>" : "conv_gemm_mt<f32>") : conv_gemm_mt_name(a);
  static const char *names[2][5] = {{"conv_gemm<f32,64x64,scalarA>", "conv_gemm<f32,128x32>", "conv_gemm<f32,128x64>", "conv_gemm<f32,64x64>", "conv_gemm<f32,128x128>"},
                                    {"conv_gemm<bf16,64x64,scalarA>", "conv_gemm<bf16,128x32>", "conv_gemm<bf16,128x64>", "conv_gemm<bf16,64x64>", "conv_gemm<bf16,128x128>"}};
  static const char *sk_names[2][3] = {{"conv_gemm_sk<f32,64x64>", "conv_gemm_sk<f32,64x32>", "conv_gemm_sk<f32,32x32>"},
                                       {"conv_gemm_sk<bf16,64x64>", "conv_gemm_sk<bf16,64x32>", "conv_gemm_sk<bf16,32x32>"}};
  static const char *fast_names[2][3] = {{"conv_gemm_fast<f32,64x64>", "conv_gemm_fast<f32,64x32>", "conv_gemm_fast<f32,32x32>"},
                                         {"conv_gemm_fast<bf16,64x64>", "conv_gemm_fast<bf16,64x32>", "conv_gemm_fast<bf16,32x32>"}};
  const long t64 = (long)((a.M + 63) / 64) * ((a.n_store + 63) / 64);
  const bool short_act = t64 < short_act_tiles() && a.K >= 256 && (a.K % 32) == 0 && (a.cin % 32) == 0 && (a.cin2 % 32) == 0;
  if (!short_act) {
    V2Plan pl;
    if (conv_gemm_v2_plan(dt, a, pl)) return conv_gemm_v2_name(dt, pl);
  }
  static const char *wp_names[2][3] = {{"conv_gemm_wp<f32,32x32>", "conv_gemm_wp<f32,32x32>", "conv_gemm_wp<f32,32x32>"},
                                       {"conv_gemm_wp<bf16,64x64>", "conv_gemm_wp<bf16,64x32>", "conv_gemm_wp<bf16,32x32>"}};
  if ((short_act || use_sk(a)) && conv_gemm_prefers_wp(a) && conv_gemm_sk_variant(a) == 2 && g_conv_gemm_force.path == 0 && conv_gemm_rs_ok(dt, a))
    return dt == F32 ? "conv_gemm_rs<x3,32x32>" : "conv_gemm_rs<bf16,32x32>";
  if ((short_act || use_sk(a)) && conv_gemm_prefers_wp(a) && conv_gemm_wp_ok(dt, a)) return wp_names[dt == F32 ? 0 : 1][conv_gemm_sk_variant(a)];
  if (short_act || use_sk(a)) return (conv_gemm_fast_ok(dt, a) ? fast_names : sk_names)[dt == F32 ? 0 : 1][conv_gemm_sk_variant(a)];
  int v = pick_variant(a);
  return v < 0 ? "conv_gemm<invalid>" : names[dt == F32 ? 0 : 1][v];
}

ConvGemmForce g_conv_gemm_force;


bool conv_gemm_emits_rowpart(int dt, const ConvGemmArgs &a) {
  if (g_conv_gemm_force.path != 0 || !conv_gemm_supported(dt, a)) return false;
  {
    ConvGemmArgs plain = a;
    plain.rowpart_out = nullptr;
    if (conv_gemm_mt_wanted(dt, plain)) {
      const bool off = a.mt_ln == 0;
      ConvGemmArgs probe = a;
      if (!probe.rowpart_out) {
        probe.rowpart_out = reinterpret_cast<float *>(16);
        probe.rowpart_nt = a.n_store / 32;
      }
      return !off && conv_gemm_mt_wanted(dt, probe);
    }
  }
  if ((a.n_store % 32) || a.n_store != a.N) return false;
  const long t64 = (long)((a.M + 63) / 64) * ((a.n_store + 63) / 64);
  const bool short_act = t64 < short_act_tiles() && a.K >= 256 && (a.K % 32) == 0 && (a.cin % 32) == 0 && (a.cin2 % 32) == 0;
  if (!(short_act || use_sk(a))) return false;
  if ((a.cin % 32) || (a.cin2 % 32) || (a.K % 32)) return false;
  if (conv_gemm_sk_variant(a) != 2) return false;
  const bool prefer_wp = conv_gemm_prefers_wp(a);
  if (prefer_wp && conv_gemm_wp_ok(dt, a)) return true;
  return conv_gemm_fast_ok(dt, a);
}

bool conv_gemm_emits_gnpart(int dt, const ConvGemmArgs &a) {
  ConvGemmArgs plain = a;
  plain.gnpart_out = nullptr;
  if (a.geom != 0 || a.Lout < 32 || !conv_gemm_emits_rowpart(dt, plain)) return false;
  return conv_gemm_prefers_wp(a) && conv_gemm_wp_ok(dt, a);
}

hipError_t launch_conv_gemm(int dt, const ConvGemmArgs &a, hipStream_t s) {
  if (!conv_gemm_supported(dt, a)) return hipErrorInvalidValue;
  if (a.src_x3 && (dt != F32 || g_conv_gemm_force.path != 0 || !conv_gemm_src_x3_ok(a))) return hipErrorInvalidValue;
  const ConvGemmForce &f = g_conv_gemm_force;
  if (f.path == 6) return launch_conv_gemm_mt(dt, a, s);
  if (f.path == 0 && conv_gemm_mt_wanted(dt, a)) return launch_conv_gemm_mt(dt, a, s);
  const long t64 = (long)((a.M + 63) / 64) * ((a.n_store + 63) / 64);
  const bool short_act = t64 < short_act_tiles() && a.K >= 256 && (a.K % 32) == 0 && (a.cin % 32) == 0 && (a.cin2 % 32) == 0;
  if (f.path == 4 || (f.path == 0 && !short_act)) {
    V2Plan pl;
    if (conv_gemm_v2_plan(dt, a, pl)) return launch_conv_gemm_v2(dt, a, pl, s);
    if (f.path == 4) return hipErrorInvalidValue;
  }
  if (f.path == 2 || f.path == 5 || (f.path == 0 && (short_act || use_sk(a)))) return launch_conv_gemm_sk(dt, a, s);
  return SF_DISPATCH_T(dt, dispatch<T>(a, s));
}

}
```

syncfusion_amd/csrc/kernels.h:

```cpp
#pragma once
#include <hip/hip_runtime.h>
#include <stdint.h>

#include <cstdlib>

namespace sf {

#ifdef SF_TUNING_HOOKS
inline const char *tune_env(const char *name) { return getenv(name); }
#else
inline const char *tune_env(const char *) { return nullptr; }
#endif

enum DType { F32 = 0, BF16 = 1, F16 = 2, F32X = 3 };
constexpr int X3_F16 = 1, X3_BF16 = 2;
inline size_t dsize(int dt) { return (dt == F32 || dt == F32X) ? 4 : 2; }
#define SF_DISPATCH_T(dt, EXPR_T)             \
  ((dt) == ::sf::F32    ? [&] { using T = float; return EXPR_T; }()   \
   : (dt) == ::sf::BF16 ? [&] { using T = ::sf::bf16; return EXPR_T; }() \
                        : [&] { using T = ::sf::f16; return EXPR_T; }())
#define SF_DISPATCH_STMT(dt, STMT)                                   \
  do {                                                               \
    if ((dt) == ::sf::F32) { using T = float; STMT; }                \
    else if ((dt) == ::sf::BF16) { using T = ::sf::bf16; STMT; }     \
    else { using T = ::sf::f16; STMT; }                              \
  } while (0)

struct Prefetch {
  const void *ptr = nullptr;
  unsigned bytes = 0;
  int wgs = 0;
};

struct ConvGemmArgs {
  Prefetch pf;
  const void *src = nullptr, *src2 = nullptr, *w = nullptr, *res = nullptr;
  const void *wfr = nullptr;
  const float *w32 = nullptr;
  const void *wx = nullptr;
  const void *wfrx = nullptr;
  int wx_mode = 1;
  int src_x3 = 0;
  int solo = 0;
  void *out = nullptr;
  const float *bias = nullptr, *gamma = nullptr, *beta = nullptr, *stats = nullptr;
  const float *badd = nullptr, *bscale = nullptr;
  int M = 0, N = 0, K = 0;
  int cin = 0, cin2 = 0, src_ld = 0, src2_ld = 0, out_ld = 0, res_ld = 0, n_store = 0;
  int geom = 0;
  int Lout = 1, Lsrc = 1, taps = 1, stride = 1, pad = 0, up_shift = 0;
  int To = 1, Ho = 1, Wo = 1, Ti = 1, Hi = 1, Wi = 1, kt = 1, kh = 1, kw = 1, st = 1, sh = 1, sw = 1, pt = 0, ph = 0, pw = 0;
  int pro = 0, G = 1, nch = 1, chunk_rows = 1;
  float eps = 1e-5f;
  int badd_ld = 0, bscale_ld = 0, act = 0, out_f32 = 0;
  float *rowpart_out = nullptr;
  int rowpart_nt = 0;
  float *gnpart_out = nullptr;
  const float *ln_colsum = nullptr;
  const float *ln_part = nullptr, *ln_ss = nullptr;
  int ln_nt = 0, ln_ss_ld = 0, res_ln = 0;
  float ln_eps = 1e-5f;
  int mt_ln = 0;
};
struct V2Plan {
  int variant = 2;
};
bool conv_gemm_v2_plan(int dt, const ConvGemmArgs &a, V2Plan &pl);
const char *conv_gemm_v2_name(int dt, const V2Plan &pl);
hipError_t launch_conv_gemm_v2(int dt, const ConvGemmArgs &a, const V2Plan &pl, hipStream_t s);
hipError_t launch_conv_gemm(int dt, const ConvGemmArgs &a, hipStream_t s);
bool conv_gemm_mt_ok(int dt, const ConvGemmArgs &a);
bool conv_gemm_prefers_mt(const ConvGemmArgs &a);
bool conv_gemm_mt_wanted(int dt, const ConvGemmArgs &a);
bool conv_gemm_src_x3_ok(const ConvGemmArgs &a);
hipError_t launch_conv_gemm_mt(int dt, const ConvGemmArgs &a, hipStream_t s);
const char *conv_gemm_mt_name(const ConvGemmArgs &a);
bool conv_gemm_emits_rowpart(int dt, const ConvGemmArgs &a);
bool conv_gemm_rs_ok(int dt, const ConvGemmArgs &a);
bool conv_gemm_rs_rows_ok(int64_t rows, int N);
hipError_t launch_conv_gemm_rs(int dt, const ConvGemmArgs &a, hipStream_t s);
hipError_t launch_pack_wfr(int dt, const void *w , int N, int K, void *out, hipStream_t s);
hipError_t launch_pack_wfrx(const float *w , int N, int K, void *out, hipStream_t s);
hipError_t launch_pack_wx(const float *w, int N, int K, void *out, hipStream_t s, int mode = 1);
hipError_t launch_pack_conv_x(const float *w, int N, int C, int taps, float *out, void *outx, int mode, hipStream_t s);
bool conv_gemm_emits_gnpart(int dt, const ConvGemmArgs &a);
bool conv_gemm_ln_ok(int dt, const ConvGemmArgs &a);
hipError_t launch_conv_gemm_ln(int dt, const ConvGemmArgs &a, hipStream_t s);
const char *conv_gemm_ln_variant_name(int dt, const ConvGemmArgs &a);
struct ConvGemmForce {
  int path = 0, tile = -1, sk = -1;
};
extern ConvGemmForce g_conv_gemm_force;
const char *conv_gemm_variant_name(int dt, const ConvGemmArgs &a);
bool conv_gemm_reads_split_only(int dt, const ConvGemmArgs &a);
const char *label_for_dtype(int dt, const char *bf16_label);
bool conv_gemm_supported(int dt, const ConvGemmArgs &a);

struct ConvThinArgs {
  const void *src = nullptr, *src2 = nullptr, *w = nullptr, *res = nullptr;
  const float *w32 = nullptr;
  void *out = nullptr;
  const float *bias = nullptr, *gamma = nullptr, *beta = nullptr, *stats_in = nullptr, *ss = nullptr, *badd = nullptr, *bscale = nullptr;
  float *stats_out = nullptr;
  int B = 0, L = 0, Ls = 0, up_shift = 0, C = 0, N = 0, C2 = 0, taps = 1;
  int src_ld = 0, src2_ld = 0, out_ld = 0, res_ld = 0, ss_ld = 0, badd_ld = 0, bscale_ld = 0;
  int pro = 0, res_self = 0, G = 1, nch_in = 1, chunk_in = 1;
  float eps = 1e-5f;
  int rw = 32, nchw = 1;
  int x3 = 0;
};
struct ThinPlan {
  int rw = 32, nchw = 1;
};
ThinPlan conv_thin_plan(int B, int L, int C);
struct ThinTailArgs {
  const void *h = nullptr, *x = nullptr, *ctx = nullptr, *w2 = nullptr, *w3 = nullptr;
  const float *w2_32 = nullptr, *w3_32 = nullptr;
  int c2real = 0;
  void *out = nullptr;
  const float *bias2 = nullptr, *bias3 = nullptr, *gamma = nullptr, *beta = nullptr, *stats_in = nullptr, *ss = nullptr, *badd = nullptr;
  float *stats_out = nullptr;
  int B = 0, L = 0, C = 0, C2 = 0, ctx_ld = 0, ss_ld = 0, badd_ld = 0, G = 1, nch_in = 1, chunk_in = 1;
  float eps_gn = 1e-5f, eps_ln = 1e-6f;
  int rw = 32, nchw = 1;
  int x3 = 0;
};
bool thin_tail_supported(int dt, const ThinTailArgs &a);
hipError_t launch_thin_tail(int dt, const ThinTailArgs &a, hipStream_t s);
bool conv_thin_supported(int dt, const ConvThinArgs &a);
hipError_t launch_conv_thin(int dt, const ConvThinArgs &a, hipStream_t s);
bool d0_enabled(int B, int L);
bool d0_conv_supported(const ConvThinArgs &a);
bool d0_tail_supported(const ThinTailArgs &a);
hipError_t launch_d0_conv(int dt, const ConvThinArgs &a, hipStream_t s);
hipError_t launch_d0_tail(int dt, const ThinTailArgs &a, hipStream_t s);

struct ConvCbArgs {
  Prefetch pf;
  const void *src = nullptr;
  const void *wp = nullptr;
  float *slab = nullptr;
  int B = 0, L = 0, C = 0, N = 0, src_ld = 0;
  int pro = 0, G = 1, nch = 1, chunk_rows = 1;
  const float *gamma = nullptr, *beta = nullptr, *stats = nullptr;
  float eps = 1e-5f;
  int kb = 1;
  int log2S = 0, log2cpg = 7;
  unsigned magicL = 0;
};
struct CbGnPlan {
  int nch = 1, chunk_rows = 8;
};
bool conv_cb_shape_ok(int dt, int B, int L, int C, int N, int G);
bool conv_cb_tile_stats_ok(int L, int C, int G);
int conv_cb_mt(int M, int N, int C);
size_t conv_cb_weight_elems(int N, int C);
hipError_t launch_pack_conv_cb(int dt, const float *w , int N, int C, void *out, hipStream_t s);
hipError_t launch_conv_cb(int dt, const ConvCbArgs &a, hipStream_t s);
CbGnPlan cb_gn_plan(int L);
hipError_t launch_cb_reduce_gn(int dt, const float *slab, int S, int B, int L, int N, const float *bias, void *out, int out_ld, int G, float *stats,
                               const CbGnPlan &gp, hipStream_t s, Prefetch pf = Prefetch());
hipError_t launch_cb_reduce_ln(int dt, const float *slab, int S, int B, int L, int C, const float *bias, const void *res, int res_ld, const float *ss,
                               int ss_ld, float eps, void *out, int out_ld, hipStream_t s, Prefetch pf = Prefetch());

hipError_t launch_conv_direct(int dt_in, int dt_out, const ConvGemmArgs &a, hipStream_t s);
bool conv_direct_supported(const ConvGemmArgs &a);

struct GnPlan {
  int nch = 1, chunk_rows = 1;
};
GnPlan gn_plan(int B, int L, int C);
hipError_t launch_gn_stats(int dt, const void *x, int ld, int B, int L, int C, int G, int nch, int chunk_rows, float *slab,
                           hipStream_t s);

hipError_t launch_gn_silu(int dt, const void *x, int ld, int B, int L, int C, int G, const float *gamma, const float *beta, float eps,
                          void *out, int out_ld, hipStream_t s, Prefetch pf = Prefetch(), bool xfmt = false);
hipError_t launch_gn_silu_ws(int dt, const void *x, int ld, int B, int L, int C, int G, const float *gamma, const float *beta, float eps, void *out,
                             int out_ld, float *slab, int64_t slab_floats, hipStream_t s);

hipError_t launch_ln_modulate(int dt, const void *x, int ld, const float *ss, int ss_ld, float eps, int B, int L, int C,
                              void *out, int out_ld, hipStream_t s, Prefetch pf = Prefetch(), bool xfmt = false );

hipError_t launch_attention(int dt, const void *q, int ldq, const void *kv, int ldkv, int B, int L, int H, int D,
                            void *out, int ldo, hipStream_t s, bool x3 = false, bool xfmt = false );

struct CrossOutItem {
  const void *w;
  const float *bias;
  int N, ldw, v_off, out_off;
};
hipError_t launch_cross_out_grouped(int dt, const CrossOutItem *items, const int2 *blocks , int nblocks,
                                    const void *v_all, int ldv, int Bt, int hd, float *out, int out_ld, hipStream_t s);
hipError_t launch_cf_to_cl(int dt, const float *x, int B, int C, int L, void *out, int ld, hipStream_t s);
hipError_t launch_cl_to_cf(int dt, const void *x, int ld, int B, int C, int L, float *out, hipStream_t s);
hipError_t launch_video_to_cl(int dt, const float *x, int N, int C, int T, int H, int W, void *out, int ld, hipStream_t s);
hipError_t launch_to_f32(int dt, const void *x, int ld, int64_t rows, int C, float *out, hipStream_t s);

hipError_t launch_time_fourier(int dt, const float *sig, const int *sig_idx, const float *w, int B, int half, void *out, int ld,
                               hipStream_t s);

hipError_t launch_vsampler_update(float *x, const float *v, const float *v_uncond, float scale, const float *sched,
                                  const int *step_idx, int64_t n, hipStream_t s);
hipError_t launch_step_select(const float *table, int ld, int *step_idx, float *cur, hipStream_t s);
hipError_t launch_spin(double microseconds, hipStream_t s);
hipError_t launch_clock_probe(double microseconds, unsigned long long *out2, hipStream_t s);
hipError_t launch_touch(const void *p, size_t bytes, int wgs, unsigned *sink, hipStream_t s);
hipError_t launch_step_advance(int *step_idx, hipStream_t s);
hipError_t launch_cfg_combine(const float *v_c, const float *v_u, float scale, float *out, int64_t n, hipStream_t s);

hipError_t launch_spatial_mean(int dt, const void *x, int ld, int NT, int HW, int C, float *out, hipStream_t s);

hipError_t launch_resample(const float *x, int R, int L, const float *bank, int orig, int nnew, int width, float *out, int Lout,
                           hipStream_t s);

hipError_t launch_cut_prefix_crop(const float *gen, const float *y, int B, int C, int L, int Lc, float *out, int *first, hipStream_t s);
hipError_t launch_onsets_to_track(const float *logits, int N, int T, const int32_t *start_frame, float frame_rate,
                                  float sample_rate, float threshold, float *track, int L, hipStream_t s);

hipError_t launch_row_sums(int dt, const void *w, int N, int K, float *out, hipStream_t s);
hipError_t launch_pack_conv(int dt, const float *w, int N, int Ctot, int c_off, int Cin, int taps, int cin_pad, const float *nscale,
                            void *out, int64_t out_row, int64_t col0, hipStream_t s);
hipError_t launch_pack_convT(int dt, const float *w, int Cin, int Cout, int f, void *out, int64_t out_row, hipStream_t s);
hipError_t launch_pack_rows(int dt, const float *in, int64_t rows, int cols, int64_t ldi, const float *cscale, void *out,
                            int64_t ldo, hipStream_t s);
hipError_t launch_fold_bias(const float *w, int N, int K, const float *v, const float *add, float *out, hipStream_t s);
size_t onset_stem_weight_elems();
hipError_t launch_onset_stem_repack(int dt, const void *w_generic, int n_real, int k_in, void *out, hipStream_t s);
hipError_t launch_onset_stem(int dt, const void *in, int NT, int H, int W, const void *wk, const float *shift, int n_real, void *out, int out_ld,
                             hipStream_t s);

bool conv_tw_ok(int dt, int cin_real, int cin_ld, int cout, int out_ld, int res_ld);
size_t conv_tw_weight_elems(int cin_real);
hipError_t launch_pack_conv_tw(int dt, const void *w , int cin_real, int cin_ld, void *out, hipStream_t s);
hipError_t launch_conv_tw(int dt, const void *in, int in_ld, int cin_real, const void *wfr, const float *bias, const void *res, int res_ld, void *out,
                          int out_ld, int N, int T, int HW, int relu, hipStream_t s);

bool conv_sp_ok(int dt, int cin_real, int cin_ld, int cout, int out_ld);
size_t conv_sp_weight_elems(int cout);
hipError_t launch_pack_conv_sp(int dt, const void *w , int cout, void *out, hipStream_t s);
hipError_t launch_conv_sp(int dt, const void *in, int in_ld, const void *wfr, const float *shift, int cout, void *out, int out_ld, int N, int T, int H,
                          int W, int relu, hipStream_t s);

hipError_t launch_frames_preprocess(const unsigned char *frames, int N, int T, int H, int W, int oh, int ow, const float *mean, const float *stdv,
                                    float *out, hipStream_t s);
struct AugClip {
  int top, left;
  int order[4];
  float factor[4];
  int mask;
  int reserved;
};
int64_t frames_augment_workspace_bytes(int N, int T, int oh, int ow);
hipError_t launch_frames_augment(const unsigned char *frames, int N, int T, int H, int W, int rh, int rw, int oh, int ow, const AugClip *table_dev,
                                 bool any_contrast, const float *mean, const float *stdv, float *out, float *part, hipStream_t s);
hipError_t launch_times_to_track(const double *times, const int *clip_of, int n_times, double sample_rate, int B, int L, float *track, hipStream_t s);

hipError_t launch_pack_dgrad(const float *w, int N, int C, int taps, int ldn, float *out, hipStream_t s, void *outx = nullptr);
hipError_t launch_pack_train(const float *w, int N, int C, int taps, float *fw, void *fwx, float *dg, void *dgx, hipStream_t s);
hipError_t launch_pack_train_many(const void *desc_dev, int n_items, int total_tiles, hipStream_t s);
int conv_wgrad_splits(int64_t rows, int C, int N, int taps);
enum { WGRAD_REDUCE_DIRECT = 0 , WGRAD_REDUCE_VEC = 1, WGRAD_REDUCE_SCALAR = 2 };
struct ConvWgradPlan {
  int family = 0;
  bool x3 = false;
  int tq = 0;
  bool single_tap = false;
  int S = 1, rps = 0;
  int reducer = WGRAD_REDUCE_DIRECT;
};
ConvWgradPlan conv_wgrad_plan(int64_t rows, int C, int N, int taps, int S, int x3);
enum { COL_SUMS_VEC4 = 0, COL_SUMS_VEC1 = 1, COL_SUMS_GENERIC = 2 };
int col_sums_variant(int cols);
hipError_t launch_conv_wgrad(const float *dy, const float *act, int B, int L, int C, int N, int taps, int pad, float *partial, int S, float *dw,
                             hipStream_t s, int x3_mode = 0, const float *bias_part = nullptr, int bias_slices = 0, float *db = nullptr,
                             bool *bias_done = nullptr);
hipError_t launch_col_sums_part(const float *x, int64_t rows, int cols, float *part, int S, hipStream_t s);
hipError_t launch_slices_reduce(const float *part, int S, int cols, float *out, hipStream_t s);
hipError_t launch_col_sums(const float *x, int64_t rows, int cols, float *part, int S, float *out, hipStream_t s);
int length_sums_slices(int B, int L);
hipError_t launch_length_sums(const float *x, const float *y, int B, int L, int C, float *part, float *out, hipStream_t s);
hipError_t launch_gn_silu_bwd(const float *x, const float *da, const float *gamma, const float *beta, int B, int L, int C, int G, float eps,
                              float *dx, float *dgb_part, float *dgb, hipStream_t s, const float *slab_in = nullptr,
                              const float *dx_add = nullptr );
int64_t gn_bwd_stats_floats(int B, int L, int C, int G);
int64_t gn_silu_bwd_ws_floats(int B, int L, int C, int G);
hipError_t launch_gn_silu_recompute(const float *x, const float *gamma, const float *beta, int B, int L, int C, int G, float eps, float *act,
                                    float *ws, hipStream_t s);
hipError_t launch_gn_bwd_stats(const float *x, int B, int L, int C, int G, float *ws, hipStream_t s);

int ln_mod_bwd_chunks(int L, int C);
hipError_t launch_ln_modulate_bwd(const float *x, const float *ss, const float *dy, float eps, int B, int L, int C, float *dx, float *dss_part,
                                  float *dss, hipStream_t s, const float *dx_add = nullptr );
hipError_t launch_attention_bwd(const float *q, const float *kv, const float *o, const float *dout, int B, int L, int H, int D, float *dq, float *dkv,
                                float *lse, float *dsum, hipStream_t s, const float *lse_fwd = nullptr, bool x3 = false);
bool attention_f32_mfma_ok(int ldq, int ldkv, int ldo, int B, int H);
hipError_t launch_attention_f32_mfma(const float *q, int ldq, const float *kv, int ldkv, int B, int L, int H, float *out, int ldo, hipStream_t s,
                                     float *lse_out, bool x3 = false, bool xfmt = false);

struct VConvGeom {
  int cin = 0, cout = 0, T = 1, Hi = 1, Wi = 1, Ho = 1, Wo = 1, kt = 1, kh = 1, kw = 1, sh = 1, sw = 1, pt = 0, ph = 0, pw = 0;
  __host__ __device__ int taps() const { return kt * kh * kw; }
};
int vconv_k(int taps, int ld);
hipError_t launch_vconv_pack_fwd(const float *w, const VConvGeom &g, int cin_ld, float *out, hipStream_t s);
hipError_t launch_vconv_fwd(const float *x, int cin_ld, const float *wpk, const VConvGeom &g, int64_t NT, float *y, int cout_ld, hipStream_t s);
hipError_t launch_vconv_dgrad_s1(const float *dy, int cout_ld, const float *w, const VConvGeom &g, int64_t NT, float *wflip, float *dx, int cin_ld,
                                 hipStream_t s);
// ... 38 lines not shown
```

syncfusion_amd/csrc/unet_engine.cpp:

```cpp
#include <algorithm>
#include <chrono>
#include <cstdio>
#include <cstdlib>
#include <cmath>
#include <cstring>
#include <exception>
#include <memory>

#include "engine_common.h"

using namespace sf;

namespace {

struct Group {
  float *gn1_g = nullptr, *gn1_b = nullptr, *gn2_g = nullptr, *gn2_b = nullptr;
  ConvW conv1, conv2, inject, qkv, attn_out, cross_out;
  float *qkv_colsum = nullptr;
  int mod_off = 0;
  bool attn = false, cross = false;
  int ca_off = 0;
  int ca_idx = 0;
};

struct Block {
  int C = 0, cin = 0, factor = 1, ctx = 0, ctx_ld = 0, up_shift = 0;
  ConvW down, up;
  bool up_transposed = false;
  int skip_off = 0, skip_cols = 0;
  std::vector<Group> down_items, up_items;
};

struct Level {
  int L = 0, C = 0;
  int64_t rows = 0;
  void *buf[3] = {nullptr, nullptr, nullptr};
  void *qkv = nullptr, *ao = nullptr, *ctx = nullptr, *act = nullptr;
  bool cb = false;
  int cb_kb = 1;
};

struct Plan {
  int B = 0, Bt = 0, L0 = 0;
  bool two = false;
  std::vector<Level> lv;
  float *xs = nullptr;
  float *x2 = nullptr, *vout = nullptr, *mod_all = nullptr, *ca_all = nullptr, *slab = nullptr, *emb2 = nullptr;
  float *sched = nullptr;
  float *sigs = nullptr;
  void *four = nullptr, *f1 = nullptr, *f2 = nullptr, *sf = nullptr, *emb_t = nullptr, *xhat_e = nullptr, *v_all = nullptr;
  int *step = nullptr;
  int nbr = 1;
  int nbr_total = 1;
  int64_t slab_stride = 0;
  int64_t slab_half = 0;
  float *rowpart = nullptr;
  int64_t rowpart_half = 0, rowpart_stride = 0;
  float *cbslab = nullptr;
  int64_t cbslab_stride = 0;
  float *gnpart = nullptr;
  int64_t gnpart_stride = 0;
  int mod_stride = 0;
  float *mod_steps = nullptr;
  int steps_cap = 0;
};

}

struct sf_unet {
  sf_unet_config cfg{};
  int dt = SF_F32;
  bool x3 = false;
  DeviceArena arena;
  float *fourier_w = nullptr;
  int half = 0, four_ld = 0, mf = 0, hd = 0;
  ConvW lin0, mlp0, mlp1, mod, wv_cat;
  int mod_cols = 0, mod_ld = 0, ca_cols = 0, ca_ld = 0, n_ca = 0;
  float *fixed_emb = nullptr;
  CrossOutItem *ca_items = nullptr;
  int2 *ca_blocks = nullptr;
  int ca_nblocks = 0;
  std::vector<Block> blocks;
  DebugTaps dbg;
  int launches = 0;
  int graph_captures = 0;
  bool listing = false;
  struct ProfRec {
    const char *label;
    double flops, bytes;
    hipEvent_t e0, e1;
    float ms;
    int depth;
  };
  bool prof_on = false;
  std::vector<ProfRec> prof;
  std::vector<hipEvent_t> ev_pool;
  size_t ev_used = 0;
  hipEvent_t get_event() {
    if (ev_used == ev_pool.size()) {
      hipEvent_t e;
      SF_HIP(hipEventCreate(&e));
      ev_pool.push_back(e);
    }
    return ev_pool[ev_used++];
  }
  std::vector<std::pair<std::string, int64_t>> names;
  bool no_ln_fusion = tune_env("SF_NO_LN_FUSION") != nullptr;
  bool no_indep_branches = tune_env("SF_NO_INDEP_BRANCHES") != nullptr;
  bool no_thin_tail = tune_env("SF_NO_THIN_TAIL") != nullptr;
  hipGraphExec_t gexec = nullptr;
  hipGraphExec_t gexec_br[8] = {};
  bool gexec_indep = false;
  struct GraphKey {
    int B = 0, L0 = 0, T = 0, nbr = 0;
    bool two = false, valid = false;
    float scale = 0.f;
    const void *ws = nullptr;
    bool operator==(const GraphKey &o) const {
      return valid && o.valid && B == o.B && L0 == o.L0 && T == o.T && nbr == o.nbr && two == o.two && scale == o.scale && ws == o.ws;
    }
  } gkey;
  struct GraphEntry {
    GraphKey key;
    hipGraphExec_t g = nullptr, br[8] = {};
    bool indep = false;
    void destroy() {
      if (g) (void)hipGraphExecDestroy(g);
      for (hipGraphExec_t &b : br)
        if (b) (void)hipGraphExecDestroy(b);
      g = nullptr;
      for (hipGraphExec_t &b : br) b = nullptr;
    }
  };
  static constexpr size_t kGraphStash = 3;
  std::vector<GraphEntry> gstash;
  void activate_graphs(const GraphKey &key) {
    if (gkey == key) return;
    GraphEntry cur;
    cur.key = gkey;
    cur.g = gexec;
    cur.indep = gexec_indep;
    for (int i = 0; i < 8; ++i) cur.br[i] = gexec_br[i];
    gexec = nullptr;
    gexec_indep = false;
    for (hipGraphExec_t &b : gexec_br) b = nullptr;
    gkey.valid = false;
    for (size_t i = 0; i < gstash.size(); ++i)
      if (gstash[i].key == key) {
        gkey = gstash[i].key;
        gexec = gstash[i].g;
        gexec_indep = gstash[i].indep;
        for (int j = 0; j < 8; ++j) gexec_br[j] = gstash[i].br[j];
        gstash.erase(gstash.begin() + i);
        break;
      }
    if (cur.key.valid && (cur.g || cur.br[0])) {
      if (gstash.size() >= kGraphStash) {
        gstash.front().destroy();
        gstash.erase(gstash.begin());
      }
      gstash.push_back(cur);
    } else {
      cur.destroy();
    }
  }
  void drop_all_graphs() {
    gkey.valid = false;
    gexec_indep = false;
    if (gexec) (void)hipGraphExecDestroy(gexec);
    gexec = nullptr;
    for (hipGraphExec_t &g : gexec_br) {
      if (g) (void)hipGraphExecDestroy(g);
      g = nullptr;
    }
    for (GraphEntry &e : gstash) e.destroy();
    gstash.clear();
  }

  hipStream_t own_stream = nullptr;
  hipEvent_t ev_in = nullptr, ev_out = nullptr;
  static constexpr int kMaxBranches = 8;
  hipStream_t bstream[kMaxBranches] = {};
  hipEvent_t ev_fork = nullptr, ev_join[kMaxBranches] = {};
  int branches_override = 0;
  static hipError_t make_branch_stream(hipStream_t *st, int branch, int nbr) {
    static const int div = [] { const char *e = tune_env("SF_BRANCH_CUMASK"); return e ? atoi(e) : 0; }();
    if (div <= 0 || nbr < 2) return hipStreamCreateWithFlags(st, hipStreamNonBlocking);
    hipDeviceProp_t prop;
    int dev = 0;
    hipError_t e = hipGetDevice(&dev);
    if (e == hipSuccess) e = hipGetDeviceProperties(&prop, dev);
    if (e != hipSuccess) return e;
// ... 302 lines not shown
        }
      }
    }
  }
  if (!u.listing && u.n_ca > 0 && !tune_env("SF_NO_CA_GROUPED")) {
    std::vector<CrossOutItem> items;
    std::vector<int2> blks;
    for (int d = 0; d < c.n_layers; ++d)
      for (int pass = 0; pass < 2; ++pass)
        for (const Group &g : (pass == 0 ? u.blocks[d].down_items : u.blocks[d].up_items)) {
          if (!g.cross || g.cross_out.direct || !g.cross_out.w) continue;
          CrossOutItem it;
          it.w = g.cross_out.w;
          it.bias = g.cross_out.bias;
          it.N = g.cross_out.N;
          it.ldw = g.cross_out.K;
          it.v_off = g.ca_idx * u.hd;
          it.out_off = g.ca_off;
          for (int c0 = 0; c0 < it.N; c0 += 64) blks.push_back(make_int2((int)items.size(), c0));
          items.push_back(it);
        }
    if ((int)items.size() == u.n_ca && u.hd <= 1024 && (u.hd % 32) == 0) {
      u.ca_items = static_cast<CrossOutItem *>(u.arena.alloc((int64_t)items.size() * sizeof(CrossOutItem)));
      u.ca_blocks = static_cast<int2 *>(u.arena.alloc((int64_t)blks.size() * sizeof(int2)));
      SF_HIP(hipMemcpyAsync(u.ca_items, items.data(), items.size() * sizeof(CrossOutItem), hipMemcpyHostToDevice, s));
      SF_HIP(hipMemcpyAsync(u.ca_blocks, blks.data(), blks.size() * sizeof(int2), hipMemcpyHostToDevice, s));
      SF_HIP(hipStreamSynchronize(s));
      u.ca_nblocks = (int)blks.size();
    }
  }
  if (!u.listing && u.x3) {
    auto split = [&](ConvW &w) {
      if (w.direct || !w.w || (w.K % 32)) return;
      w.wx = u.arena.alloc((int64_t)w.N * w.K * 4);
      SF_HIP(launch_pack_wx(static_cast<const float *>(w.w), w.N, w.K, w.wx, s));
      if ((w.K % 64) == 0 && w.K <= 1280 && (w.N % 32) == 0 && (w.cin % 16) == 0 && (w.cin2 % 16) == 0) {
        w.wfrx = u.arena.alloc((int64_t)w.N * w.K * 4);
        SF_HIP(launch_pack_wfrx(static_cast<const float *>(w.w), w.N, w.K, w.wfrx, s));
      }
    };
    for (ConvW *w : {&u.lin0, &u.mlp0, &u.mlp1, &u.mod, &u.wv_cat}) split(*w);
    for (Block &b : u.blocks) {
      split(b.down);
      split(b.up);
      for (int pass = 0; pass < 2; ++pass)
        for (Group &g : (pass == 0 ? b.down_items : b.up_items))
          for (ConvW *w : {&g.conv1, &g.conv2, &g.inject, &g.qkv, &g.attn_out, &g.cross_out}) split(*w);
    }
  }
  if (!u.listing) SF_HIP(hipStreamSynchronize(s));
}

constexpr int kSchedSteps = 1024;

Plan make_plan(const sf_unet &u, Workspace &ws, int B, int L0, bool two, int num_steps) {
  const sf_unet_config &c = u.cfg;
  Plan p;
  p.B = B;
  p.Bt = two ? 2 * B : B;
  p.L0 = L0;
  p.two = two;
  int64_t stride = 1;
  for (int d = 0; d < c.n_layers; ++d) stride *= c.factors[d];
  if (B < 1 || L0 < 1 || L0 % stride) fail(SF_ERR_SHAPE, "L0=%d must be a positive multiple of the U-Net stride %lld", L0, (long long)stride);
  const size_t es = dsize(u.dt);
  p.lv.resize(c.n_layers);
  int L = L0;
  int64_t slab_floats = 16;
  for (int d = 0; d < c.n_layers; ++d) {
    Level &l = p.lv[d];
    L /= c.factors[d];
    l.L = L;
    l.C = c.channels[d];
    l.rows = (int64_t)p.Bt * L;
    for (int i = 0; i < 3; ++i) l.buf[i] = ws.alloc(l.rows * l.C * es);
    l.act = ws.alloc(l.rows * l.C * es);
    if (c.attentions[d]) {
      l.qkv = ws.alloc(l.rows * 3 * u.hd * es);
      l.ao = ws.alloc(l.rows * u.hd * es);
    }
    l.ctx = ws.alloc(l.rows * u.blocks[d].ctx_ld * es);
  }
  {
    static const int two_max = [] {
      const char *e = tune_env("SF_TWO_BRANCH_MAX");
      return e ? atoi(e) : 128;
    }();
    int want = u.branches_override > 0 ? u.branches_override : ((p.Bt >= 4 && p.Bt <= two_max) ? 2 : 1);
    if (want > sf_unet::kMaxBranches) want = sf_unet::kMaxBranches;
    while (want > 1 && p.Bt % want) --want;
    p.nbr = u.dbg.buf ? 1 : want;
    p.nbr_total = p.nbr;
    int64_t one = (int64_t)(p.Bt / p.nbr) * 32 * c.resnet_groups * 2;
    for (int d = 0; d < c.n_layers; ++d) {
      const ThinPlan tp = conv_thin_plan(p.Bt / p.nbr, p.lv[d].L, p.lv[d].C);
      one = std::max<int64_t>(one, (int64_t)(p.Bt / p.nbr) * tp.nchw * c.resnet_groups * 2);
    }
    p.slab_half = align_up(one, 64);
    p.slab_stride = 2 * p.slab_half;
    slab_floats = p.slab_stride * p.nbr;
  }
  const int64_t n0 = (int64_t)p.Bt * L0 * c.in_channels;
  p.x2 = ws.alloc_n<float>(n0);
  p.vout = ws.alloc_n<float>(n0);
  p.xs = ws.alloc_n<float>(n0);
  p.mod_all = ws.alloc_n<float>((int64_t)p.Bt * u.mod_ld);
  p.mod_stride = u.mod_ld;
  p.steps_cap = num_steps > 1 ? num_steps : 0;
  p.ca_all = ws.alloc_n<float>((int64_t)p.Bt * u.ca_ld);
  p.slab = ws.alloc_n<float>(slab_floats);
  {
    int64_t one = 64;
    for (int d = 0; d < c.n_layers; ++d)
      if (p.lv[d].C % 32 == 0) one = std::max<int64_t>(one, p.lv[d].rows / p.nbr * (p.lv[d].C / 32) * 2);
    p.rowpart_half = align_up(one, 64);
    p.rowpart_stride = 2 * p.rowpart_half;
    p.rowpart = ws.alloc_n<float>(p.rowpart_stride * p.nbr);
  }
  {
    static const int cb_max_rows = [] {
      const char *e = tune_env("SF_CB_MAX_ROWS");
      return e ? atoi(e) : 1408;
    }();
    static const double cb_max_slab_mb = [] {
      const char *e = tune_env("SF_CB_MAX_SLAB_MB");
      return e ? atof(e) : 12.0;
    }();
    static const int cb_min_c = [] {
      const char *e = tune_env("SF_CB_MIN_C");
      return e ? atoi(e) : 256;
    }();
    int64_t need = 0, need_gp = 0;
    for (int d = 0; d < c.n_layers; ++d) {
      Level &l = p.lv[d];
      const int bt = p.Bt / p.nbr;
      const int64_t rows = (int64_t)bt * l.L;
      const Block &b = u.blocks[d];
      const bool have_w = !b.down_items.empty() && b.down_items[0].conv1.wcb != nullptr;
      const bool shape_ok = have_w && l.C >= cb_min_c && rows <= cb_max_rows && conv_cb_shape_ok(u.x3 ? (int)F32X : u.dt, bt, l.L, l.C, l.C, c.resnet_groups) &&
                            cb_gn_plan(l.L).nch <= 32 && (int64_t)bt * 32 * c.resnet_groups * 2 <= p.slab_half;
      const double slab1 = (double)(l.C / 128) * rows * l.C * 4.0;
      static const bool no_kb2 = tune_env("SF_CB_NO_KB2") != nullptr;
      static const double cb_max_slab2_mb = [] {
        const char *e = tune_env("SF_CB_MAX_SLAB2_MB");
        return e ? atof(e) : 12.0;
      }();
      l.cb = false;
      l.cb_kb = 1;
      if (shape_ok && slab1 <= cb_max_slab_mb * 1048576.0) l.cb = true;
      else if (shape_ok && !u.x3 && !no_kb2 && (l.C / 128) % 2 == 0 && l.C / c.resnet_groups >= 32 && slab1 * 0.5 <= cb_max_slab2_mb * 1048576.0) {
        l.cb = true;
        l.cb_kb = 2;
      }
      if (l.cb) need = std::max<int64_t>(need, (int64_t)(l.C / 128 / l.cb_kb) * rows * l.C);
      if (l.cb) need_gp = std::max<int64_t>(need_gp, ((rows + 31) / 32) * (l.C / 32) * 4);
    }
    p.cbslab_stride = align_up(need, 64);
    p.cbslab = need ? ws.alloc_n<float>(p.cbslab_stride * p.nbr) : nullptr;
    p.gnpart_stride = align_up(need_gp, 64);
    p.gnpart = need_gp ? ws.alloc_n<float>(p.gnpart_stride * p.nbr) : nullptr;
  }
  p.emb2 = ws.alloc_n<float>((int64_t)p.Bt * c.embedding_features);
  p.emb_t = ws.alloc((int64_t)p.Bt * c.embedding_features * es);
  p.xhat_e = ws.alloc((int64_t)p.Bt * c.embedding_features * es);
  p.v_all = ws.alloc((int64_t)p.Bt * (u.n_ca > 0 ? u.n_ca : 1) * u.hd * es);
  const int64_t ns = std::max<int64_t>(num_steps > 0 ? num_steps : 1, kSchedSteps);
  p.step = ws.alloc_n<int>(16);
  p.sched = ws.alloc_n<float>(4 * ns);
  p.sigs = ws.alloc_n<float>(ns + p.Bt);
  if (p.steps_cap) p.mod_steps = ws.alloc_n<float>((int64_t)p.steps_cap * u.mod_ld);
  const int64_t frows = std::max<int64_t>(p.Bt, p.steps_cap);
  p.four = ws.alloc(frows * u.four_ld * es);
  p.f1 = ws.alloc(frows * u.mf * es);
  p.f2 = ws.alloc(frows * u.mf * es);
  p.sf = ws.alloc(frows * u.mf * es);
  return p;
}

struct Exec {
  sf_unet &u;
  Plan &p;
  hipStream_t s;
  const void *stats_of = nullptr;
  const void *gnpart_of = nullptr;
  bool up_gnpart = false;
  int cur_depth = -1;

  template <class F> void timed(const char *label, double flops, double bytes, F &&f) {
#ifdef SF_TUNING_HOOKS
    {
      static const std::vector<std::string> skip = [] {
        std::vector<std::string> v;
        if (const char *e = tune_env("SF_SKIP_LABELS")) {
          std::string all(e);
          size_t a = 0;
          while (a <= all.size()) {
            const size_t b = all.find(',', a);
            const std::string t = all.substr(a, b == std::string::npos ? std::string::npos : b - a);
            if (!t.empty()) v.push_back(t);
            if (b == std::string::npos) break;
            a = b + 1;
          }
        }
        return v;
      }();
      for (const std::string &t : skip)
        if (strncmp(label, t.c_str(), t.size()) == 0) return;
    }
#endif
    ++u.launches;
    if (!u.prof_on) {
      f();
      return;
    }
    hipEvent_t e0 = u.get_event(), e1 = u.get_event();
    SF_HIP(hipEventRecord(e0, s));
    f();
    SF_HIP(hipEventRecord(e1, s));
    u.prof.push_back({label, flops, bytes, e0, e1, 0.f, cur_depth});
  }

  Prefetch pf_for(const ConvW &w, int host_wgs, int64_t rows = -1) const {
    const bool rs = (w.wfr || w.wfrx) && rows >= 0 && conv_gemm_rs_rows_ok(rows, w.N);
    return pf_bytes(w.direct ? nullptr : (rs ? (w.wfrx ? w.wfrx : w.wfr) : (w.wx ? w.wx : w.w)), (size_t)w.N * w.K * dsize(u.dt), host_wgs);
  }
  Prefetch pf_cb(const ConvW &w, int host_wgs) const { return pf_bytes(w.wcb, conv_cb_weight_elems(w.N, w.cin) * dsize(u.dt), host_wgs); }
  Prefetch pf_bytes(const void *ptr, size_t bytes, int host_wgs) const {
    static const bool off = tune_env("SF_NO_PREFETCH") != nullptr;
    Prefetch pf;
    static const int host_max = [] {
      const char *e = tune_env("SF_PF_HOST_MAX");
      return e ? atoi(e) : 1024;
    }();
    if (off || !ptr || host_wgs > host_max) return pf;
    if (bytes < (64u << 10) || bytes > 0x7FFFFFF0ull) return pf;
    pf.ptr = ptr;
    pf.bytes = (unsigned)bytes;
    static const int cap = [] {
      const char *e = tune_env("SF_PF_WGS");
      return e && atoi(e) > 0 ? atoi(e) : 224;
    }();
    static const int mult = [] {
      const char *e = tune_env("SF_PF_MULT");
      return e && atoi(e) > 0 ? atoi(e) : 1;
    }();
    pf.wgs = std::max(std::min(48, cap), std::min(cap, mult * (256 - host_wgs)));
    return pf;
  }

  bool wants_gnpart(int d) const {
    static const bool off = tune_env("SF_NO_CB_TILESTATS") != nullptr;
    if (off || d < 0 || d >= (int)p.lv.size()) return false;
    const Level &l = p.lv[d];
    return l.cb && p.gnpart && conv_cb_tile_stats_ok(l.L, l.C, u.cfg.resnet_groups);
  }
  bool arm_gnpart(const ConvW &w, ConvGemmArgs &a, int d) const {
    if (!wants_gnpart(d)) return false;
    a.gnpart_out = p.gnpart;
    if (conv_gemm_emits_gnpart(u.dt, filled(w, a))) return true;
    a.gnpart_out = nullptr;
    return false;
  }

  ConvGemmArgs filled(const ConvW &w, ConvGemmArgs a) const {
    a.w = w.w;
    a.wfr = w.wfr;
    a.wx = w.wx;
    a.wfrx = w.wfrx;
    a.solo = p.nbr_total <= 1 ? 1 : 0;
    a.bias = w.bias;
    a.N = w.N;
    a.K = w.K;
    a.cin = w.cin;
    a.cin2 = w.cin2;
    a.taps = w.taps;
    if (a.n_store == 0) a.n_store = w.N;
    return a;
  }

  void conv(const ConvW &w, ConvGemmArgs a0, int dt_in, int dt_out, bool ln = false) {
    ConvGemmArgs a = filled(w, a0);
    const double kreal = w.kreal > 0 ? w.kreal : w.K;
    const double es_in = dsize(dt_in), es_out = a.out_f32 ? 4.0 : (double)dsize(dt_out);
    const double flops = 2.0 * a.M * w.N * kreal;
    const double src_rows = (double)a.M / a.Lout * a.Lsrc;
    const double bytes = src_rows * (kreal / (w.taps > 0 ? w.taps : 1)) * es_in + (double)a.M * w.N * es_out * (a.res ? 2 : 1) +
                         (double)w.N * kreal * (w.direct ? 4.0 : (double)dsize(u.dt));
    if (w.direct) timed("conv_direct", flops, bytes, [&] { SF_HIP(launch_conv_direct(dt_in, dt_out, a, s)); });
    else {
      static const int touch = [] {
        const char *e = tune_env("SF_TOUCH");
        return e ? atoi(e) : 0;
      }();
      if (touch > 0 && !u.prof_on) SF_HIP(launch_touch(w.w, (size_t)w.N * w.K * dsize(u.dt), touch, reinterpret_cast<unsigned *>(p.step + 8), s));
      if (dt_in != u.dt || (dt_out != u.dt && !a.out_f32)) fail(SF_ERR_INVALID, "internal: dtype mismatch on the MFMA path");
      if (ln) timed(conv_gemm_ln_variant_name(u.dt, a), flops + 8.0 * a.M * a.cin, bytes,
                    [&] { SF_HIP(launch_conv_gemm_ln(u.dt, a, s)); });
      else timed(conv_gemm_variant_name(u.dt, a), flops, bytes, [&] { SF_HIP(launch_conv_gemm(u.dt, a, s)); });
    }
  }

  void dense(const ConvW &w, const void *src, int src_ld, int rows, void *out, int out_ld, int act, bool out_f32, int col0 = 0,
             int ncols = -1) {
    ConvGemmArgs a;
    a.src = src;
    a.src_ld = src_ld;
    a.M = rows;
    a.Lout = a.Lsrc = 1;
    a.out = out;
    a.out_ld = out_ld;
    a.act = act;
    a.out_f32 = out_f32 ? 1 : 0;
    (void)col0;
    (void)ncols;
    conv(w, a, u.dt, out_f32 ? F32 : u.dt);
  }

  void gn(const void *x, int d, int C) {
    const Level &l = p.lv[d];
    GnPlan gp = gn_plan(p.Bt, l.L, C);
    timed("gn_stats", 3.0 * l.rows * C, (double)l.rows * C * dsize(u.dt),
          [&] { SF_HIP(launch_gn_stats(u.dt, x, C, p.Bt, l.L, C, u.cfg.resnet_groups, gp.nch, gp.chunk_rows, p.slab, s)); });
  }

  void group(const Group &g, int d, void *&cur, void *&tA, void *&tB, const std::string &tapname, const Group *next = nullptr) {
    const Level &l = p.lv[d];
    const Block &b = u.blocks[d];
    const int C = l.C, G = u.cfg.resnet_groups;
    if (group_thin(g, d, cur, tA, tB)) {
      if (!g.attn) {
        u.dbg.tap(tapname, u.dt, cur, C, l.rows, C, s);
        return;
      }
    } else {
    const bool fuse_act = C <= 64;
    GnPlan gp = gn_plan(p.Bt, l.L, C);
    auto conv3 = [&](const ConvW &w, const void *in, void *out, const float *gam, const float *bet, const void *res, float *rowpart,
                     const ConvW *next = nullptr) {
      ConvGemmArgs a;
      if (next) a.pf = pf_for(*next, (int)((l.rows + 31) / 32) * ((C + 31) / 32), l.rows);
      if (rowpart) {
        a.rowpart_out = rowpart;
        a.rowpart_nt = C / 32;
      }
      if (fuse_act) {
        gn(in, d, C);
        a.src = in;
        a.pro = 1;
        a.G = G;
        a.nch = gp.nch;
        a.chunk_rows = gp.chunk_rows;
        a.stats = p.slab;
        a.gamma = gam;
        a.beta = bet;
        a.eps = 1e-5f;
      } else {
        a.src = l.act;
      }
      a.src_ld = C;
      a.M = (int)l.rows;
      a.Lout = a.Lsrc = l.L;
      a.stride = 1;
      a.pad = 1;
      a.out = out;
      a.out_ld = C;
      a.res = res;
      a.res_ld = C;
      if (!fuse_act) {
        const bool xf = u.x3 && (C % 32) == 0 && conv_gemm_src_x3_ok(filled(w, a));
        timed("gn_silu", 12.0 * l.rows * C, 3.0 * l.rows * C * dsize(u.dt),
              [&] { SF_HIP(launch_gn_silu(u.dt, in, C, p.Bt, l.L, C, G, gam, bet, 1e-5f, l.act, C, s, pf_for(w, p.Bt * G), xf)); });
        a.src_x3 = xf ? 1 : 0;
      }
      conv(w, a, u.dt, u.dt);
    };
    float *rp_y = p.rowpart, *rp_z = p.rowpart + p.rowpart_half;
    auto inject_args = [&](const void *src, void *out) {
      ConvGemmArgs a;
      a.src = src;
      a.src_ld = C;
      a.src2 = l.ctx;
      a.src2_ld = b.ctx_ld;
      a.M = (int)l.rows;
      a.Lout = a.Lsrc = l.L;
      a.out = out;
      a.out_ld = C;
      a.res = src;
      a.res_ld = C;
      if (g.cross && !g.attn) {
        a.badd = p.ca_all + g.ca_off;
        a.badd_ld = u.ca_ld;
      }
      return a;
    };
    auto qkv_args = [&](const void *src) {
      ConvGemmArgs a;
      a.src = src;
      a.src_ld = C;
      a.M = (int)l.rows;
      a.Lout = a.Lsrc = l.L;
      a.out = l.qkv;
      a.out_ld = 3 * u.hd;
      return a;
    };
    bool fuse_mod = false;
    static const int ln_fuse_maxc = [] {
      const char *e = tune_env("SF_LN_FUSE_MAXC");
      return e ? atoi(e) : 512;
    }();
    if (!fuse_act && C % 32 == 0 && C <= ln_fuse_maxc && !u.no_ln_fusion) {
      ConvGemmArgs pc;
      pc.src = l.act;
      pc.src_ld = C;
      pc.M = (int)l.rows;
      pc.Lout = pc.Lsrc = l.L;
      pc.pad = 1;
      pc.out = tB;
      pc.out_ld = C;
      pc.res = cur;
      pc.res_ld = C;
      ConvGemmArgs pi = inject_args(tB, tA);
      pi.ln_part = rp_y;
      pi.ln_nt = C / 32;
      pi.ln_ss = p.mod_all + g.mod_off;
      pi.ln_ss_ld = p.mod_stride;
      pi.ln_eps = 1e-6f;
      pi.res_ln = 1;
      fuse_mod = conv_gemm_emits_rowpart(u.dt, filled(g.conv2, pc)) && conv_gemm_ln_ok(u.dt, filled(g.inject, pi));
    }
    const bool use_cb = l.cb && !fuse_act && g.conv1.wcb && g.conv2.wcb && g.conv1.bias && g.conv2.bias && p.cbslab;
    bool fuse_attn = false;
    if (g.attn && C % 32 == 0 && !u.no_ln_fusion) {
      ConvGemmArgs pq = qkv_args(tB);
      pq.ln_part = rp_z;
      pq.ln_nt = C / 32;
      pq.ln_eps = 1e-5f;
      pq.ln_colsum = g.qkv_colsum;
      ConvGemmArgs pi = inject_args(tA, tB);
      const bool inj_emits = (fuse_mod && !use_cb) ? true : conv_gemm_emits_rowpart(u.dt, filled(g.inject, pi));
      fuse_attn = inj_emits && conv_gemm_ln_ok(u.dt, filled(g.qkv, pq));
    }
    if (use_cb) {
      const int bt = p.Bt, kb = l.cb_kb, S = C / 128 / kb;
      const double es = dsize(u.dt), rc = (double)l.rows * C;
      const double cflops = 2.0 * rc * 3 * C, cbytes = 2.0 * rc * es + 3.0 * C * C * es;
      const int mt = kb == 2 ? std::min(2, conv_cb_mt((int)l.rows, C, C / 2)) : conv_cb_mt((int)l.rows, C, C);
      const int cwgs = (int)((l.rows + 32 * mt - 1) / (32 * mt)) * (C / 128) * S;
      const CbGnPlan cgp = cb_gn_plan(l.L);
      const int cbdt = u.x3 ? (int)F32X : u.dt;
      ConvCbArgs a;
      a.src_ld = C;
      a.wp = g.conv1.wcb;
      a.slab = p.cbslab;
      a.B = bt;
      a.L = l.L;
      a.C = a.N = C;
      a.kb = kb;
      a.G = G;
      a.eps = 1e-5f;
      a.pf = pf_cb(g.conv2, cwgs);
      if (gnpart_of == cur && wants_gnpart(d)) {
        a.src = cur;
        a.pro = 2;
        a.stats = p.gnpart;
        a.gamma = g.gn1_g;
        a.beta = g.gn1_b;
        timed("conv_cb", cflops + 12.0 * rc, cbytes, [&] { SF_HIP(launch_conv_cb(cbdt, a, s)); });
      } else {
        timed("gn_silu", 12.0 * rc, 3.0 * rc * es,
              [&] { SF_HIP(launch_gn_silu(u.dt, cur, C, bt, l.L, C, G, g.gn1_g, g.gn1_b, 1e-5f, l.act, C, s, pf_cb(g.conv1, bt * G))); });
        a.src = l.act;
        timed("conv_cb", cflops, cbytes, [&] { SF_HIP(launch_conv_cb(cbdt, a, s)); });
      }
      gnpart_of = nullptr;
      timed("cb_reduce_gn", 4.0 * rc, 2.0 * rc * es, [&] {
        SF_HIP(launch_cb_reduce_gn(u.dt, p.cbslab, S, bt, l.L, C, g.conv1.bias, tA, C, G, p.slab, cgp, s, pf_cb(g.conv2, bt * cgp.nch * (C / 128))));
      });
      a.src = tA;
      a.wp = g.conv2.wcb;
      a.pro = 1;
      a.nch = cgp.nch;
      a.chunk_rows = cgp.chunk_rows;
      a.stats = p.slab;
      a.gamma = g.gn2_g;
      a.beta = g.gn2_b;
      a.pf = pf_for(g.inject, cwgs, l.rows);
      timed("conv_cb", cflops + 12.0 * rc, cbytes, [&] { SF_HIP(launch_conv_cb(cbdt, a, s)); });
      timed("cb_reduce_ln", 12.0 * rc, 3.0 * rc * es, [&] {
        SF_HIP(launch_cb_reduce_ln(u.dt, p.cbslab, S, bt, l.L, C, g.conv2.bias, cur, C, p.mod_all + g.mod_off, p.mod_stride, 1e-6f, tA, C, s,
                                   pf_for(g.inject, (int)(l.rows * (C / 4) / 256), l.rows)));
      });
      stats_of = nullptr;
      ConvGemmArgs ai = inject_args(tA, tB);
      if (fuse_attn) {
        ai.rowpart_out = rp_z;
        ai.rowpart_nt = C / 32;
      }
      if (g.attn) ai.pf = pf_for(g.qkv, (int)((l.rows + 31) / 32) * (C / 32), l.rows);
      else if (next && arm_gnpart(g.inject, ai, d)) gnpart_of = tB;
      conv(g.inject, ai, u.dt, u.dt);
    } else {
    conv3(g.conv1, cur, tA, g.gn1_g, g.gn1_b, nullptr, nullptr);
    conv3(g.conv2, tA, tB, g.gn2_g, g.gn2_b, cur, fuse_mod ? rp_y : nullptr, fuse_mod ? &g.inject : nullptr);
    if (fuse_mod) {
      ConvGemmArgs a = inject_args(tB, tA);
      a.ln_part = rp_y;
      a.ln_nt = C / 32;
      a.ln_ss = p.mod_all + g.mod_off;
      a.ln_ss_ld = p.mod_stride;
      a.ln_eps = 1e-6f;
      a.res_ln = 1;
      if (fuse_attn) {
        a.rowpart_out = rp_z;
        a.rowpart_nt = C / 32;
      }
      if (g.attn) a.pf = pf_for(g.qkv, (int)((l.rows + 31) / 32) * (C / 32), l.rows);
      conv(g.inject, a, u.dt, u.dt, true);
      std::swap(tA, tB);
    } else {
      timed("ln_modulate", 8.0 * l.rows * C, 2.0 * l.rows * C * dsize(u.dt),
            [&] { SF_HIP(launch_ln_modulate(u.dt, tB, C, p.mod_all + g.mod_off, p.mod_stride, 1e-6f, p.Bt, l.L, C, tA, C, s,
                                            pf_for(g.inject, (int)(l.rows / 4), l.rows))); });
      ConvGemmArgs a = inject_args(tA, tB);
      if (fuse_attn) {
        a.rowpart_out = rp_z;
        a.rowpart_nt = C / 32;
      }
      if (g.attn) a.pf = pf_for(g.qkv, (int)((l.rows + 31) / 32) * (C / 32), l.rows);
      conv(g.inject, a, u.dt, u.dt);
    }
    }
    if (g.attn) {
      if (fuse_attn) {
        ConvGemmArgs a = qkv_args(tB);
        a.ln_part = rp_z;
        a.ln_nt = C / 32;
        a.ln_eps = 1e-5f;
        a.ln_colsum = g.qkv_colsum;
        a.pf = pf_for(g.attn_out, (int)((l.rows + 31) / 32) * (3 * u.hd / 32), l.rows);
        conv(g.qkv, a, u.dt, u.dt, true);
      } else {
        ConvGemmArgs aq = qkv_args(tA);
        const bool xf = u.x3 && (C % 32) == 0 && conv_gemm_src_x3_ok(filled(g.qkv, aq));
        timed("ln_modulate", 6.0 * l.rows * C, 2.0 * l.rows * C * dsize(u.dt),
              [&] { SF_HIP(launch_ln_modulate(u.dt, tB, C, nullptr, 0, 1e-5f, p.Bt, l.L, C, tA, C, s, Prefetch(), xf)); });
        aq.src_x3 = xf ? 1 : 0;
        conv(g.qkv, aq, u.dt, u.dt);
      }
      attention_tail(g, d, cur, tB, next);
      u.dbg.tap(tapname, u.dt, cur, C, l.rows, C, s);
      return;
    } else {
      void *o = cur;
      cur = tB;
      tB = tA;
      tA = o;
      u.dbg.tap(tapname, u.dt, cur, C, l.rows, C, s);
      return;
    }
    }
    if (g.attn) {
      timed("ln_modulate", 6.0 * l.rows * C, 2.0 * l.rows * C * dsize(u.dt),
            [&] { SF_HIP(launch_ln_modulate(u.dt, tB, C, nullptr, 0, 1e-5f, p.Bt, l.L, C, tA, C, s)); });
      {
        ConvGemmArgs a;
        a.src = tA;
        a.src_ld = C;
        a.M = (int)l.rows;
        a.Lout = a.Lsrc = l.L;
        a.out = l.qkv;
        a.out_ld = 3 * u.hd;
        conv(g.qkv, a, u.dt, u.dt);
      }
      attention_tail(g, d, cur, tB, next);
    } else {
      void *o = cur;
      cur = tB;
      tB = tA;
      tA = o;
    }
    u.dbg.tap(tapname, u.dt, cur, C, l.rows, C, s);
  }

  void attention_tail(const Group &g, int d, void *out, const void *z, const Group *next = nullptr) {
    const Level &l = p.lv[d];
    const int C = l.C;
    const size_t es = dsize(u.dt);
    ConvGemmArgs a;
    a.src = l.ao;
    a.src_ld = u.hd;
    a.M = (int)l.rows;
    a.Lout = a.Lsrc = l.L;
    a.out = out;
    a.out_ld = C;
    a.res = z;
    a.res_ld = C;
    if (g.cross) {
      a.badd = p.ca_all + g.ca_off;
      a.badd_ld = u.ca_ld;
    }
    const bool xf = u.x3 && (u.hd % 32) == 0 && attention_f32_mfma_ok(3 * u.hd, 3 * u.hd, u.hd, p.Bt, u.cfg.attention_heads) &&
                    conv_gemm_src_x3_ok(filled(g.attn_out, a));
    timed("attention", 4.0 * p.Bt * (double)l.L * l.L * u.hd, 4.0 * l.rows * u.hd * es, [&] {
      SF_HIP(launch_attention(u.dt, l.qkv, 3 * u.hd, static_cast<char *>(l.qkv) + (size_t)u.hd * es, 3 * u.hd, p.Bt, l.L,
                              u.cfg.attention_heads, u.cfg.attention_features, l.ao, u.hd, s, u.x3, xf));
    });
    a.src_x3 = xf ? 1 : 0;
    gnpart_of = nullptr;
    if (next && arm_gnpart(g.attn_out, a, d)) {
      gnpart_of = out;
      if (next->conv1.wcb) a.pf = pf_cb(next->conv1, (int)((l.rows + 31) / 32) * (C / 32));
    }
    conv(g.attn_out, a, u.dt, u.dt);
  }

  bool group_thin(const Group &g, int d, void *&cur, void *&tA, void *&tB) {
    const Level &l = p.lv[d];
    const Block &b = u.blocks[d];
    const int C = l.C, G = u.cfg.resnet_groups;
    if (g.conv1.cin != C || g.inject.cin != C) return false;
    const void *w1 = g.conv1.direct ? g.conv1.wt : g.conv1.w, *w2 = g.conv2.direct ? g.conv2.wt : g.conv2.w;
    const void *w3 = g.inject.direct ? g.inject.wt : g.inject.w;
    if (!w1 || !w2 || !w3) return false;
    const ThinPlan tp = conv_thin_plan(p.Bt, l.L, C);
    ConvThinArgs base;
    base.B = p.Bt;
    base.L = base.Ls = l.L;
    base.C = base.N = C;
    base.G = G;
    base.rw = tp.rw;
    base.nchw = tp.nchw;
    base.nch_in = tp.nchw;
    base.chunk_in = tp.rw;
    base.src_ld = base.out_ld = base.res_ld = C;
    base.x3 = u.x3 ? 1 : 0;
    ConvThinArgs a1 = base, a3 = base;
    a1.taps = 3;
    a1.pro = 1;
    a3.taps = 1;
    a3.pro = 2;
    a3.C2 = g.inject.direct ? pad_to(g.inject.cin2, 8) : g.inject.cin2;
    if (a3.C2 > b.ctx_ld) return false;
    if (!conv_thin_supported(u.dt, a1) || !conv_thin_supported(u.dt, a3)) return false;
    float *sA = p.slab, *sB = p.slab + p.slab_half;
    const double es = dsize(u.dt), rc = (double)l.rows * C;
    if (stats_of != cur)
      timed("gn_stats", 3.0 * rc, rc * es, [&] { SF_HIP(launch_gn_stats(u.dt, cur, C, p.Bt, l.L, C, G, tp.nchw, tp.rw, sA, s)); });
    {
      ConvThinArgs a = a1;
      a.src = cur;
      a.w = w1;
      if (g.conv1.direct) a.w32 = static_cast<const float *>(g.conv1.w);
// ... 763 lines not shown
```

Baseline: 533.2 steps/s.

## Add direct-epilogue channel-block conv path for small C=128 resnet blocks

Adds new epilogue modes to the channel-block conv kernel. Mode 1 writes bias-added output directly and computes GroupNorm chunk stats in-kernel. Mode 2 fuses bias, residual add, LayerNorm and scale/shift modulation into the second conv's epilogue. This replaces the slab write plus separate reduce/LN pass for C=128 layers with up to 2816 rows. It also lets the inject GEMM use the short-activation path at K>=128. The cost is extra register and LDS pressure, and the path only covers a narrow set of shapes.

```diff
diff --git a/include/syncfusion_amd.h b/include/syncfusion_amd.h
--- a/include/syncfusion_amd.h
+++ b/include/syncfusion_amd.h
@@ -200,6 +200,11 @@
                         const float *gn1_b, const float *gn2_g, const float *gn2_b, int groups, float eps_gn, const float *scale_shift,
                         float eps_ln, int B, int L, int C, int kb , void *h_out, void *m_out,
                         void *ws, int64_t ws_bytes, void *stream);
+int64_t sf_op_resnet_mod_cbd_workspace_bytes(int B, int L, int C, int C2);
+int sf_op_resnet_mod_cbd(int dtype, const void *x, const float *w1, const float *b1, const float *w2, const float *b2, const float *gn1_g,
+                         const float *gn1_b, const float *gn2_g, const float *gn2_b, int groups, float eps_gn, const float *scale_shift,
+                         float eps_ln, int B, int L, int C, const float *w_inj, const float *b_inj, const void *ctx, int ctx_ld, int C2,
+                         const float *badd, void *h_out, void *m_out, void *z_out, float *stats_out, void *ws, int64_t ws_bytes, void *stream);
 int64_t sf_op_inject_prenorm_proj_workspace_bytes(int B, int L, int C, int C2, int N);
 int sf_op_inject_prenorm_proj(int dtype, const void *m, const void *ctx, const float *w_inj, const float *b_inj, const float *gamma,
                               const float *beta, float eps, const float *w_q, int B, int L, int C, int C2, int N, void *z_out, void *q_out,
diff --git a/syncfusion_amd/_lib.py b/syncfusion_amd/_lib.py
--- a/syncfusion_amd/_lib.py
+++ b/syncfusion_amd/_lib.py
@@ -125,6 +125,9 @@
     "sf_op_inject_prenorm_proj": (_I, [_I, _P, _P, _P, _P, _P, _P, _F, _P, _I, _I, _I, _I, _I, _P, _P, _P, _P, _L, _P]),
     "sf_op_resnet_mod_cb_workspace_bytes": (_L, [_I, _I, _I]),
     "sf_op_resnet_mod_cb": (_I, [_I, _P, _P, _P, _P, _P, _P, _P, _P, _P, _I, _F, _P, _F, _I, _I, _I, _I, _P, _P, _P, _L, _P]),
+    "sf_op_resnet_mod_cbd_workspace_bytes": (_L, [_I, _I, _I, _I]),
+    "sf_op_resnet_mod_cbd": (_I, [_I, _P, _P, _P, _P, _P, _P, _P, _P, _P, _I, _F, _P, _F, _I, _I, _I, _P, _P, _P, _I, _I, _P, _P, _P, _P, _P, _P,
+                                  _L, _P]),
     "sf_bench_conv_cb": (_I, [_I, _I, _I, _I, _I, _I, _I, _I, C.POINTER(C.c_float)]),
     "sf_op_ln_modulate": (_I, [_I, _P, _P, _F, _I, _I, _I, _P, _P]),
     "sf_op_attention": (_I, [_I, _P, _P, _I, _I, _I, _I, _P, _P]),
diff --git a/syncfusion_amd/csrc/capi_misc.cpp b/syncfusion_amd/csrc/capi_misc.cpp
--- a/syncfusion_amd/csrc/capi_misc.cpp
+++ b/syncfusion_amd/csrc/capi_misc.cpp
@@ -548,6 +548,113 @@
   a.eps = eps_gn;
   SF_HIP(launch_conv_cb(dtype, a, s));
   SF_HIP(launch_cb_reduce_ln(adt, slab, S, B, L, C, b2, x, C, scale_shift, 2 * C, eps_ln, m_out, C, s));
+  return SF_OK;
+  SF_API_END
+}
+
+int64_t sf_op_resnet_mod_cbd_workspace_bytes(int B, int L, int C, int C2) {
+  if (B < 1 || L < 1 || C < 1 || C2 < 0) return -1;
+  Workspace dry(nullptr, 0);
+  const int64_t M = (int64_t)B * L;
+  dry.alloc(2 * (int64_t)C * C * 3 * 2);
+  dry.alloc(M * C * 2);
+  dry.alloc(M * C * 2);
+  dry.alloc(M * C * 2);
+  dry.alloc((int64_t)B * 32 * 64 * 2 * 4);
+  dry.alloc((int64_t)C * (C + C2) * 2);
+  return dry.used();
+}
+
+int sf_op_resnet_mod_cbd(int dtype, const void *x, const float *w1, const float *b1, const float *w2, const float *b2, const float *gn1_g,
+                         const float *gn1_b, const float *gn2_g, const float *gn2_b, int groups, float eps_gn, const float *scale_shift, float eps_ln,
+                         int B, int L, int C, const float *w_inj, const float *b_inj, const void *ctx, int ctx_ld, int C2, const float *badd,
+                         void *h_out, void *m_out, void *z_out, float *stats_out, void *ws, int64_t ws_bytes, void *stream) {
+  SF_API_BEGIN
+  if (!x || !w1 || !b1 || !w2 || !b2 || !gn1_g || !gn1_b || !gn2_g || !gn2_b || !ws) fail(SF_ERR_INVALID, "null argument");
+  if (!m_out && !(w_inj && z_out)) fail(SF_ERR_INVALID, "no output requested");
+  if (w_inj && (!b_inj || !z_out || C2 < 0 || (C2 > 0 && (!ctx || ctx_ld < C2)))) fail(SF_ERR_INVALID, "InjectChannels operands incomplete");
+  if (groups < 1 || groups > 64 || !conv_cb_direct_ok(dtype, B, L, C, C, groups))
+    fail(SF_ERR_UNSUPPORTED, "shape outside the direct channel-block epilogues' coverage (16-bit, C = 128, L a multiple of 32, L <= 1024)");
+  const int64_t M = (int64_t)B * L;
+  ConvGemmArgs ai;
+  if (w_inj) {
+    if (C2 % 32 || ctx_ld % 8) fail(SF_ERR_UNSUPPORTED, "C2 must be a multiple of 32 and ctx_ld of 8");
+    ai.src_ld = C;
+    ai.src2 = C2 ? ctx : nullptr;
+    ai.src2_ld = ctx_ld;
+    ai.bias = b_inj;
+    ai.M = (int)M;
+    ai.N = ai.n_store = C;
+    ai.K = C + C2;
+    ai.cin = C;
+    ai.cin2 = C2;
+    ai.taps = 1;
+    ai.Lout = ai.Lsrc = L;
+    ai.out = z_out;
+    ai.out_ld = C;
+    ai.res_ld = C;
+    ai.short_k = 1;
+    if (badd) {
+      ai.badd = badd;
+      ai.badd_ld = C;
+    }
+  }
+  const int64_t need = sf_op_resnet_mod_cbd_workspace_bytes(B, L, C, w_inj ? C2 : 0);
+  if (need < 0 || ws_bytes < need) fail(SF_ERR_WORKSPACE, "workspace too small: need %lld bytes", (long long)need);
+  hipStream_t s = static_cast<hipStream_t>(stream);
+  Workspace wk(ws, ws_bytes);
+  const int64_t es = 2;
+  char *wp = static_cast<char *>(wk.alloc(2 * (int64_t)C * C * 3 * es));
+  void *wp1 = wp, *wp2 = wp + (int64_t)C * C * 3 * es;
+  void *act = wk.alloc(M * C * es);
+  void *h = h_out ? h_out : wk.alloc(M * C * es);
+  void *m = m_out ? m_out : wk.alloc(M * C * es);
+  float *stats = stats_out ? stats_out : static_cast<float *>(wk.alloc((int64_t)B * 32 * 64 * 2 * 4));
+  if (w_inj) {
+    void *wi = wk.alloc((int64_t)C * (C + C2) * es);
+    ai.w = wi;
+    ai.src = ai.res = m;
+    if (!conv_gemm_supported(dtype, ai)) fail(SF_ERR_UNSUPPORTED, "InjectChannels shape outside the GEMM kernels' coverage");
+    SF_HIP(launch_pack_rows(dtype, w_inj, C, C + C2, C + C2, nullptr, wi, C + C2, s));
+  }
+  SF_HIP(launch_pack_conv_cb(dtype, w1, C, C, wp1, s));
+  SF_HIP(launch_pack_conv_cb(dtype, w2, C, C, wp2, s));
+  SF_HIP(launch_gn_silu(dtype, x, C, B, L, C, groups, gn1_g, gn1_b, eps_gn, act, C, s));
+  ConvCbArgs a;
+  a.src = act;
+  a.src_ld = C;
+  a.wp = wp1;
+  a.B = B;
+  a.L = L;
+  a.C = a.N = C;
+  a.G = groups;
+  const CbGnPlan gp = cb_gn_plan(L);
+  a.nch = gp.nch;
+  a.chunk_rows = gp.chunk_rows;
+  a.epi = 1;
+  a.out = h;
+  a.out_ld = C;
+  a.bias = b1;
+  a.stats_out = stats;
+  SF_HIP(launch_conv_cb(dtype, a, s));
+  a.src = h;
+  a.wp = wp2;
+  a.pro = 1;
+  a.stats = stats;
+  a.gamma = gn2_g;
+  a.beta = gn2_b;
+  a.eps = eps_gn;
+  a.epi = 2;
+  a.out = m;
+  a.bias = b2;
+  a.stats_out = nullptr;
+  a.res = x;
+  a.res_ld = C;
+  a.ss = scale_shift;
+  a.ss_ld = 2 * C;
+  a.eps_ln = eps_ln;
+  SF_HIP(launch_conv_cb(dtype, a, s));
+  if (w_inj) SF_HIP(launch_conv_gemm(dtype, ai, s));
   return SF_OK;
   SF_API_END
 }
diff --git a/syncfusion_amd/csrc/conv_cb.hip b/syncfusion_amd/csrc/conv_cb.hip
--- a/syncfusion_amd/csrc/conv_cb.hip
+++ b/syncfusion_amd/csrc/conv_cb.hip
@@ -40,9 +40,11 @@
   return make_float2(mean, rsqrtf(sum8_dpp(s2) * rn + eps));
 }
 
-template <typename T, int MT, bool PRO, int KB>
+template <typename T, int MT, bool PRO, int KB, int EPI = 0>
 __global__ __launch_bounds__(256) void conv_cb_kernel(const ConvCbArgs a, const int mtiles, const unsigned bytes_src) {
   using frag = typename Frag16<T>::type;
+  using v4 = T __attribute__((ext_vector_type(4)));
+  static_assert(EPI == 0 || (KB == 1 && MT <= 2), "direct epilogues: one channel block, at most two row tiles");
   constexpr int KCW = KC * KB, PITCHW = KCW + 8, TPR = KCW / 8, RPP = 256 / TPR;
   constexpr int BM = 32 * MT, PR = BM + 2, NV = (PR + RPP - 1) / RPP;
   __shared__ __attribute__((aligned(16))) T panel[PR * PITCHW];
@@ -116,6 +118,31 @@
     for (int s = 0; s < 24; ++s) wf[blk * 24 + s] = wp[s * 64 + lane];
   }
   __builtin_amdgcn_sched_barrier(0);
+  const int fr = lane & 31, fh = lane >> 5;
+  const int ec0 = wave * 32 + 4 * fh;
+  f32x4 eb[4], esc[MT][4], esh[MT][4];
+  v4 er[MT][4];
+  if constexpr (EPI != 0) {
+#pragma unroll
+    for (int g = 0; g < 4; ++g) eb[g] = *reinterpret_cast<const f32x4 *>(a.bias + ec0 + 8 * g);
+  }
+  if constexpr (EPI == 2) {
+    const float *ssp = a.ss ? a.ss : a.bias;
+    const int sh_off = a.ss ? a.N : 0;
+#pragma unroll
+    for (int t = 0; t < MT; ++t) {
+      const int m = min(r0 + t * 32 + fr, M - 1);
+      const T *rp = static_cast<const T *>(a.res) + (size_t)m * a.res_ld + ec0;
+      const float *sp = ssp + (a.ss ? (size_t)divL(min(r0 + t * 32, M - 1)) * a.ss_ld : 0) + ec0;
+#pragma unroll
+      for (int g = 0; g < 4; ++g) {
+        er[t][g] = *reinterpret_cast<const v4 *>(rp + 8 * g);
+        esc[t][g] = *reinterpret_cast<const f32x4 *>(sp + 8 * g);
+        esh[t][g] = *reinterpret_cast<const f32x4 *>(sp + sh_off + 8 * g);
+      }
+    }
+  }
+  __builtin_amdgcn_sched_barrier(0);
   if constexpr (PRO) {
 #pragma unroll
     for (int rd = 0; rd < NRD; ++rd)
@@ -150,7 +177,6 @@
     }
   }
   __syncthreads();
-  const int fr = lane & 31, fh = lane >> 5;
   bool ok0[MT], ok2[MT];
 #pragma unroll
   for (int t = 0; t < MT; ++t) {
@@ -177,6 +203,7 @@
           if (tap == 2) af = ok2[t] ? af : zf;
           acc[t] = mfma32x16(wf[blk * 24 + tap * 8 + ks], af, acc[t]);
         }
+  if constexpr (EPI == 0) {
   float *sl = a.slab + (size_t)cb * M * a.N + nt * 128 + wave * 32 + 4 * fh;
 #pragma unroll
   for (int t = 0; t < MT; ++t) {
@@ -188,6 +215,150 @@
         *reinterpret_cast<f32x4 *>(sl + (unsigned)(m * a.N + 8 * g)) = v;
       }
     }
+  }
+  } else if constexpr (EPI == 1) {
+  __syncthreads();
+  T *tile = panel;
+  float *red = reinterpret_cast<float *>(panel + BM * 128);
+  float *gmean = red + 64;
+  static_assert(BM * 128 * sizeof(T) + 72 * sizeof(float) <= PR * PITCHW * sizeof(T), "tile + reduction scratch fit the panel");
+  T *outp = static_cast<T *>(a.out) + ec0;
+#pragma unroll
+  for (int t = 0; t < MT; ++t) {
+    const int m = r0 + t * 32 + fr;
+    const bool live = r0 + t * 32 < M;
+#pragma unroll
+    for (int g = 0; g < 4; ++g) {
+      v4 o;
+#pragma unroll
+      for (int e = 0; e < 4; ++e) o[e] = from_f<T>(acc[t][4 * g + e] + eb[g][e]);
+      if (live) *reinterpret_cast<v4 *>(outp + (size_t)m * a.out_ld + 8 * g) = o;
+      *reinterpret_cast<v4 *>(tile + (t * 32 + fr) * 128 + ec0 + 8 * g) = o;
+    }
+  }
+  __syncthreads();
+  {
+    const int R = a.chunk_rows, P = R >> 3;
+    const int cq = tid & 31, rr = tid >> 5;
+    const int cpg = 1 << a.log2cpg, span = cpg >> 2, gpb = KC >> a.log2cpg;
+    auto group_total = [&](float tt, int k) {
+      for (int off = 1; off < span; off <<= 1) tt += __shfl_xor(tt, off, 64);
+      tt += __shfl_xor(tt, 32, 64);
+      if (lane < 32 && (cq % span) == 0) red[(wave * 8 + cq / span) * 2 + k] = tt;
+      __syncthreads();
+      float x = 0.f;
+      if (tid < gpb) {
+#pragma unroll
+        for (int w = 0; w < 4; ++w) x += red[(w * 8 + tid) * 2 + k];
+      }
+      return x;
+    };
+    for (int ch = 0; ch < BM / R; ++ch) {
+      const int m0 = r0 + ch * R;
+      float xs[4][4];
+      float s1 = 0.f;
+#pragma unroll
+      for (int pp = 0; pp < 4; ++pp)
+        if (pp < P) {
+          const v4 v = *reinterpret_cast<const v4 *>(tile + (ch * R + pp * 8 + rr) * 128 + cq * 4);
+#pragma unroll
+          for (int e = 0; e < 4; ++e) {
+            xs[pp][e] = to_f(v[e]);
+            s1 += xs[pp][e];
+          }
+        }
+      const float a1 = group_total(s1, 0);
+      if (tid < gpb) gmean[tid] = a1 / ((float)R * (float)cpg);
+      __syncthreads();
+      const float mu = gmean[cq / span];
+      float s2 = 0.f;
+#pragma unroll
+      for (int pp = 0; pp < 4; ++pp)
+        if (pp < P) {
+#pragma unroll
+          for (int e = 0; e < 4; ++e) {
+            const float d = xs[pp][e] - mu;
+            s2 = fmaf(d, d, s2);
+          }
+        }
+      const float a2 = group_total(s2, 1);
+      if (tid < gpb && m0 < M) {
+        const int clip = divL(m0), kc = (m0 - clip * a.L) / R;
+        float *o = a.stats_out + ((size_t)(clip * a.nch + kc) * gpb + tid) * 2;
+        o[0] = gmean[tid];
+        o[1] = a2;
+      }
+      __syncthreads();
+    }
+  }
+  } else {
+  __syncthreads();
+  float *red = reinterpret_cast<float *>(panel);
+  static_assert(2 * BM * 32 * sizeof(float) <= PR * PITCHW * sizeof(T), "the quad sums of both passes fit the panel");
+  T *outp = static_cast<T *>(a.out) + ec0;
+  const int myslot = (fh * 4 + wave) ^ (fr & 7);
+  auto row_total = [&](const float *rowp) {
+    float tot[2];
+#pragma unroll
+    for (int h = 0; h < 2; ++h) {
+      f32x4 v[4];
+#pragma unroll
+      for (int w = 0; w < 4; ++w) v[w] = *reinterpret_cast<const f32x4 *>(rowp + (((h * 4 + w) ^ (fr & 7)) << 2));
+      float u[4];
+#pragma unroll
+      for (int g = 0; g < 4; ++g) u[g] = (v[0][g] + v[2][g]) + (v[1][g] + v[3][g]);
+      tot[h] = (u[0] + u[2]) + (u[1] + u[3]);
+    }
+    return tot[0] + tot[1];
+  };
+  float y[MT][16];
+#pragma unroll
+  for (int t = 0; t < MT; ++t) {
+    f32x4 p;
+#pragma unroll
+    for (int g = 0; g < 4; ++g) {
+#pragma unroll
+      for (int e = 0; e < 4; ++e) y[t][4 * g + e] = (acc[t][4 * g + e] + eb[g][e]) + to_f(er[t][g][e]);
+      p[g] = (y[t][4 * g] + y[t][4 * g + 1]) + (y[t][4 * g + 2] + y[t][4 * g + 3]);
+    }
+    *reinterpret_cast<f32x4 *>(red + (t * 32 + fr) * 32 + (myslot << 2)) = p;
+  }
+  __syncthreads();
+  float mean[MT];
+#pragma unroll
+  for (int t = 0; t < MT; ++t) {
+    mean[t] = row_total(red + (t * 32 + fr) * 32) / 128.0f;
+    f32x4 q;
+#pragma unroll
+    for (int g = 0; g < 4; ++g) {
+      q[g] = 0.f;
+#pragma unroll
+      for (int e = 0; e < 4; ++e) {
+        const float d = y[t][4 * g + e] - mean[t];
+        q[g] = fmaf(d, d, q[g]);
+      }
+    }
+    *reinterpret_cast<f32x4 *>(red + (BM + t * 32 + fr) * 32 + (myslot << 2)) = q;
+  }
+  __syncthreads();
+#pragma unroll
+  for (int t = 0; t < MT; ++t) {
+    const int m = r0 + t * 32 + fr;
+    const float rstd = rsqrtf(row_total(red + (BM + t * 32 + fr) * 32) / 128.0f + a.eps_ln);
+    if (m < M) {
+#pragma unroll
+      for (int g = 0; g < 4; ++g) {
+        v4 o;
+#pragma unroll
+        for (int e = 0; e < 4; ++e) {
+          float z = (y[t][4 * g + e] - mean[t]) * rstd;
+          if (a.ss) z = fmaf(z, 1.0f + esc[t][g][e], esh[t][g][e]);
+          o[e] = from_f<T>(z);
+        }
+        *reinterpret_cast<v4 *>(outp + (size_t)m * a.out_ld + 8 * g) = o;
+      }
+    }
+  }
   }
 }
 
@@ -559,6 +730,12 @@
   return ((L + 30) / 32 + 1) * (cpg / 32) <= 32;
 }
 
+bool conv_cb_direct_ok(int dt, int B, int L, int C, int N, int G) {
+  if (dt != BF16 && dt != F16) return false;
+  if (C != KC || N != KC || (L % 32) || L / 32 > 32) return false;
+  return conv_cb_shape_ok(dt, B, L, C, N, G);
+}
+
 int conv_cb_mt(int M, int N, int C) {
   static const int forced = [] {
     const char *e = tune_env("SF_CB_MT");
@@ -585,18 +762,27 @@
   if (a0.pro == 2 && !conv_cb_tile_stats_ok(a0.L, a0.C, a0.G)) return hipErrorInvalidValue;
   ConvCbArgs a = a0;
   if (dt == F32X && a.kb == 2) return hipErrorInvalidValue;
+  if (a.epi) {
+    if (!((a.epi == 1 && a.pro == 0) || (a.epi == 2 && a.pro == 1)) || a.kb == 2) return hipErrorInvalidValue;
+    if (!conv_cb_direct_ok(dt, a.B, a.L, a.C, a.N, a.G) || a.G < 1) return hipErrorInvalidValue;
+    if (!a.out || !a.bias || (a.out_ld % 4) || a.out_ld < a.N) return hipErrorInvalidValue;
+    if (a.epi == 1 && !a.stats_out) return hipErrorInvalidValue;
+    if (a.epi == 2 && (!a.res || (a.res_ld % 4) || a.res_ld < a.N)) return hipErrorInvalidValue;
+    if (a.epi == 2 && a.ss && ((a.ss_ld % 4) || (reinterpret_cast<uintptr_t>(a.ss) % 16))) return hipErrorInvalidValue;
+    if ((a.chunk_rows != 8 && a.chunk_rows != 16 && a.chunk_rows != 32) || a.nch * a.chunk_rows != a.L || a.nch > 32) return hipErrorInvalidValue;
+  }
   const int kb = a.kb == 2 ? 2 : 1;
   const int M = a.B * a.L, S = a.C / KC / kb;
   if (kb == 2 && ((a.C / KC) % 2 || (a.pro && a.C / a.G < 32))) return hipErrorInvalidValue;
   a.log2S = 0;
   while ((1 << a.log2S) < S) ++a.log2S;
-  const int cpg = a.pro ? a.C / a.G : KC;
+  const int cpg = (a.pro || a.epi == 1) ? a.C / a.G : KC;
   a.log2cpg = 0;
   while ((1 << a.log2cpg) < cpg) ++a.log2cpg;
   if ((1 << a.log2S) != S || (1 << a.log2cpg) != cpg) return hipErrorInvalidValue;
   a.magicL = (unsigned)((0x100000000ull + (unsigned)a.L - 1) / (unsigned)a.L);
   int mt = kb == 2 ? std::min(2, conv_cb_mt(M, a.N, a.C / 2)) : conv_cb_mt(M, a.N, a.C);
-  if (dt == F32X) mt = std::min(mt, 2);
+  if (dt == F32X || a.epi) mt = std::min(mt, 2);
   const int mtiles = (M + 32 * mt - 1) / (32 * mt), nws = (a.N / 128) * S;
   const int pf_rows = (a.pf.ptr && a.pf.bytes >= 16 && a.pf.wgs > 0) ? (a.pf.wgs + nws - 1) / nws : 0;
   a.pf.wgs = pf_rows * nws;
@@ -610,6 +796,22 @@
       if (mt == 1) hipLaunchKernelGGL((conv_cb_x3_kernel<1, false>), grid, dim3(256), 0, s, a, mtiles, bytes_src);
       else hipLaunchKernelGGL((conv_cb_x3_kernel<2, false>), grid, dim3(256), 0, s, a, mtiles, bytes_src);
     }
+    return hipGetLastError();
+  }
+  if (a.epi) {
+#define SF_CBD(T, MT)                                                                                                          \
+  do {                                                                                                                         \
+    if (a.epi == 1) hipLaunchKernelGGL((conv_cb_kernel<T, MT, false, 1, 1>), grid, dim3(256), 0, s, a, mtiles, bytes_src);     \
+    else hipLaunchKernelGGL((conv_cb_kernel<T, MT, true, 1, 2>), grid, dim3(256), 0, s, a, mtiles, bytes_src);                 \
+  } while (0)
+    if (dt == BF16) {
+      if (mt == 1) SF_CBD(bf16, 1);
+      else SF_CBD(bf16, 2);
+    } else {
+      if (mt == 1) SF_CBD(f16, 1);
+      else SF_CBD(f16, 2);
+    }
+#undef SF_CBD
     return hipGetLastError();
   }
 #define SF_CB2(T, MT, KB_)                                                                                                \
diff --git a/syncfusion_amd/csrc/conv_gemm.hip b/syncfusion_amd/csrc/conv_gemm.hip
--- a/syncfusion_amd/csrc/conv_gemm.hip
+++ b/syncfusion_amd/csrc/conv_gemm.hip
@@ -450,7 +450,7 @@
   static const char *fast_names[2][3] = {{"conv_gemm_fast<f32,64x64>", "conv_gemm_fast<f32,64x32>", "conv_gemm_fast<f32,32x32>"},
                                          {"conv_gemm_fast<bf16,64x64>", "conv_gemm_fast<bf16,64x32>", "conv_gemm_fast<bf16,32x32>"}};
   const long t64 = (long)((a.M + 63) / 64) * ((a.n_store + 63) / 64);
-  const bool short_act = t64 < short_act_tiles() && a.K >= 256 && (a.K % 32) == 0 && (a.cin % 32) == 0 && (a.cin2 % 32) == 0;
+  const bool short_act = t64 < short_act_tiles() && a.K >= (a.short_k ? 128 : 256) && (a.K % 32) == 0 && (a.cin % 32) == 0 && (a.cin2 % 32) == 0;
   if (!short_act) {
     V2Plan pl;
     if (conv_gemm_v2_plan(dt, a, pl)) return conv_gemm_v2_name(dt, pl);
@@ -485,7 +485,7 @@
   }
   if ((a.n_store % 32) || a.n_store != a.N) return false;
   const long t64 = (long)((a.M + 63) / 64) * ((a.n_store + 63) / 64);
-  const bool short_act = t64 < short_act_tiles() && a.K >= 256 && (a.K % 32) == 0 && (a.cin % 32) == 0 && (a.cin2 % 32) == 0;
+  const bool short_act = t64 < short_act_tiles() && a.K >= (a.short_k ? 128 : 256) && (a.K % 32) == 0 && (a.cin % 32) == 0 && (a.cin2 % 32) == 0;
   if (!(short_act || use_sk(a))) return false;
   if ((a.cin % 32) || (a.cin2 % 32) || (a.K % 32)) return false;
   if (conv_gemm_sk_variant(a) != 2) return false;
@@ -508,7 +508,7 @@
   if (f.path == 6) return launch_conv_gemm_mt(dt, a, s);
   if (f.path == 0 && conv_gemm_mt_wanted(dt, a)) return launch_conv_gemm_mt(dt, a, s);
   const long t64 = (long)((a.M + 63) / 64) * ((a.n_store + 63) / 64);
-  const bool short_act = t64 < short_act_tiles() && a.K >= 256 && (a.K % 32) == 0 && (a.cin % 32) == 0 && (a.cin2 % 32) == 0;
+  const bool short_act = t64 < short_act_tiles() && a.K >= (a.short_k ? 128 : 256) && (a.K % 32) == 0 && (a.cin % 32) == 0 && (a.cin2 % 32) == 0;
   if (f.path == 4 || (f.path == 0 && !short_act)) {
     V2Plan pl;
     if (conv_gemm_v2_plan(dt, a, pl)) return launch_conv_gemm_v2(dt, a, pl, s);
diff --git a/syncfusion_amd/csrc/kernels.h b/syncfusion_amd/csrc/kernels.h
--- a/syncfusion_amd/csrc/kernels.h
+++ b/syncfusion_amd/csrc/kernels.h
@@ -53,6 +53,7 @@
   int pro = 0, G = 1, nch = 1, chunk_rows = 1;
   float eps = 1e-5f;
   int badd_ld = 0, bscale_ld = 0, act = 0, out_f32 = 0;
+  int short_k = 0;
   float *rowpart_out = nullptr;
   int rowpart_nt = 0;
   float *gnpart_out = nullptr;
@@ -145,6 +146,13 @@
   const float *gamma = nullptr, *beta = nullptr, *stats = nullptr;
   float eps = 1e-5f;
   int kb = 1;
+  int epi = 0;
+  void *out = nullptr;
+  const float *bias = nullptr, *ss = nullptr;
+  const void *res = nullptr;
+  float *stats_out = nullptr;
+  int out_ld = 0, res_ld = 0, ss_ld = 0;
+  float eps_ln = 1e-6f;
   int log2S = 0, log2cpg = 7;
   unsigned magicL = 0;
 };
@@ -153,6 +161,7 @@
 };
 bool conv_cb_shape_ok(int dt, int B, int L, int C, int N, int G);
 bool conv_cb_tile_stats_ok(int L, int C, int G);
+bool conv_cb_direct_ok(int dt, int B, int L, int C, int N, int G);
 int conv_cb_mt(int M, int N, int C);
 size_t conv_cb_weight_elems(int N, int C);
 hipError_t launch_pack_conv_cb(int dt, const float *w , int N, int C, void *out, hipStream_t s);
diff --git a/syncfusion_amd/csrc/unet_engine.cpp b/syncfusion_amd/csrc/unet_engine.cpp
--- a/syncfusion_amd/csrc/unet_engine.cpp
+++ b/syncfusion_amd/csrc/unet_engine.cpp
@@ -38,6 +38,7 @@
   void *qkv = nullptr, *ao = nullptr, *ctx = nullptr, *act = nullptr;
   bool cb = false;
   int cb_kb = 1;
+  bool cbd = false;
 };
 
 struct Plan {
@@ -646,6 +647,10 @@
         l.cb = true;
         l.cb_kb = 2;
       }
+      static const bool no_cbd = tune_env("SF_NO_CB_DIRECT") != nullptr;
+      static const int cbd_max_rows = 2816;
+      l.cbd = !l.cb && !no_cbd && !u.x3 && have_w && l.C == 128 && rows <= cbd_max_rows && conv_cb_direct_ok(u.dt, bt, l.L, l.C, l.C, c.resnet_groups) &&
+              (int64_t)bt * 32 * c.resnet_groups * 2 <= p.slab_half;
       if (l.cb) need = std::max<int64_t>(need, (int64_t)(l.C / 128 / l.cb_kb) * rows * l.C);
       if (l.cb) need_gp = std::max<int64_t>(need_gp, ((rows + 31) / 32) * (l.C / 32) * 4);
     }
@@ -923,6 +928,8 @@
       fuse_mod = conv_gemm_emits_rowpart(u.dt, filled(g.conv2, pc)) && conv_gemm_ln_ok(u.dt, filled(g.inject, pi));
     }
     const bool use_cb = l.cb && !fuse_act && g.conv1.wcb && g.conv2.wcb && g.conv1.bias && g.conv2.bias && p.cbslab;
+    const bool use_cbd = l.cbd && !use_cb && !fuse_act && g.conv1.wcb && g.conv2.wcb && g.conv1.bias && g.conv2.bias && g.conv1.cin == C &&
+                         (g.mod_off % 4) == 0 && (p.mod_stride % 4) == 0;
     bool fuse_attn = false;
     if (g.attn && C % 32 == 0 && !u.no_ln_fusion) {
       ConvGemmArgs pq = qkv_args(tB);
@@ -931,7 +938,8 @@
       pq.ln_eps = 1e-5f;
       pq.ln_colsum = g.qkv_colsum;
       ConvGemmArgs pi = inject_args(tA, tB);
-      const bool inj_emits = (fuse_mod && !use_cb) ? true : conv_gemm_emits_rowpart(u.dt, filled(g.inject, pi));
+      pi.short_k = use_cbd ? 1 : 0;
+      const bool inj_emits = (fuse_mod && !use_cb && !use_cbd) ? true : conv_gemm_emits_rowpart(u.dt, filled(g.inject, pi));
       fuse_attn = inj_emits && conv_gemm_ln_ok(u.dt, filled(g.qkv, pq));
     }
     if (use_cb) {
@@ -992,6 +1000,60 @@
       }
       if (g.attn) ai.pf = pf_for(g.qkv, (int)((l.rows + 31) / 32) * (C / 32), l.rows);
       else if (next && arm_gnpart(g.inject, ai, d)) gnpart_of = tB;
+      conv(g.inject, ai, u.dt, u.dt);
+    } else if (use_cbd) {
+      const int bt = p.Bt;
+      const double es = dsize(u.dt), rc = (double)l.rows * C;
+      const double cflops = 2.0 * rc * 3 * C, cbytes = 2.0 * rc * es + 3.0 * C * C * es;
+      const int mt = std::min(2, conv_cb_mt((int)l.rows, C, C));
+      const int cwgs = (int)((l.rows + 32 * mt - 1) / (32 * mt));
+      timed("gn_silu", 12.0 * rc, 3.0 * rc * es,
+            [&] { SF_HIP(launch_gn_silu(u.dt, cur, C, bt, l.L, C, G, g.gn1_g, g.gn1_b, 1e-5f, l.act, C, s, pf_cb(g.conv1, bt * G))); });
+      ConvCbArgs a;
+      a.src = l.act;
+      a.src_ld = C;
+      a.wp = g.conv1.wcb;
+      a.B = bt;
+      a.L = l.L;
+      a.C = a.N = C;
+      a.G = G;
+      a.eps = 1e-5f;
+      const CbGnPlan cgp = cb_gn_plan(l.L);
+      a.nch = cgp.nch;
+      a.chunk_rows = cgp.chunk_rows;
+      a.epi = 1;
+      a.out = tA;
+      a.out_ld = C;
+      a.bias = g.conv1.bias;
+      a.stats_out = p.slab;
+      a.pf = pf_cb(g.conv2, cwgs);
+      timed("conv_cb_gn", cflops + 6.0 * rc, cbytes, [&] { SF_HIP(launch_conv_cb(u.dt, a, s)); });
+      a.src = tA;
+      a.wp = g.conv2.wcb;
+      a.pro = 1;
+      a.stats = p.slab;
+      a.gamma = g.gn2_g;
+      a.beta = g.gn2_b;
+      a.epi = 2;
+      a.out = l.act;
+      a.bias = g.conv2.bias;
+      a.stats_out = nullptr;
+      a.res = cur;
+      a.res_ld = C;
+      a.ss = p.mod_all + g.mod_off;
+      a.ss_ld = p.mod_stride;
+      a.eps_ln = 1e-6f;
+      a.pf = pf_for(g.inject, cwgs, l.rows);
+      timed("conv_cb_ln", cflops + 24.0 * rc, cbytes + rc * es, [&] { SF_HIP(launch_conv_cb(u.dt, a, s)); });
+      stats_of = nullptr;
+      gnpart_of = nullptr;
+      ConvGemmArgs ai = inject_args(l.act, tB);
+      ai.short_k = 1;
+      if (fuse_attn) {
+        ai.rowpart_out = rp_z;
+        ai.rowpart_nt = C / 32;
+      }
+      if (g.attn) ai.pf = pf_for(g.qkv, (int)((l.rows + 31) / 32) * (C / 32), l.rows);
       conv(g.inject, ai, u.dt, u.dt);
     } else {
     conv3(g.conv1, cur, tA, g.gn1_g, g.gn1_b, nullptr, nullptr);
```

Result: faster. 540.4 steps/s (median of 6 runs) (+1.3%).
